# julilili42/hockey-env

Measured on NVIDIA B200. Metric: env-steps/sec, higher is better.
Workload: dtype f32

## Files before the change

hockey_env_b200/csrc/hk_lib.cu:

```cuda
#include <cuda_runtime.h>
#include <cstdio>
#include <cstdlib>
#include <cstring>
#include <algorithm>
#include <string>

#include "../../include/hockey_b200.h"
#include "hk_tick.cuh"
#if !defined(HK_TU_INLINE)
#include "hk_actor.cuh"
#endif

using namespace hk;

namespace {

__constant__ Scene c_scene;

thread_local std::string g_err;
int fail(int code, const std::string& msg) {
  g_err = msg;
  return code;
}
#define HK_CUDA(call)                                                                           \
// ... 30 lines not shown
  for (int k = 0; k < CORE_GROUPS; ++k) {
    float4 v = __ldcs(&core[(int64_t)k * n + i]);
    g[k] = F4{v.x, v.y, v.z, v.w};
  }
  groupsToEnv(g, e);
}
__device__ __forceinline__ void storeEnv(float4* __restrict__ core, int64_t n, int64_t i, const Env& e) {
  F4 g[CORE_GROUPS];
  envToGroups(e, g);
#pragma unroll
  for (int k = 0; k < CORE_GROUPS; ++k) __stcs(&core[(int64_t)k * n + i], make_float4(g[k].x, g[k].y, g[k].z, g[k].w));
}

__device__ __forceinline__ void flushInt(double* gstats, int slot, int v, int lane) {
  if (!__any_sync(0xffffffffu, v != 0)) return;
  int s = __reduce_add_sync(0xffffffffu, v);
  if (lane == 0 && s != 0) atomicAdd(&gstats[slot], (double)s);
}
__device__ __forceinline__ double warpSumD(double v) {
  for (int o = 16; o > 0; o >>= 1) v += __shfl_down_sync(0xffffffffu, v, o);
  return v;
}
constexpr int kStatsRows = 64;
__device__ __forceinline__ double* statsRow(double* gstats) { return gstats + HK_STATS_DIM * (blockIdx.x & (kStatsRows - 1)); }
__device__ __forceinline__ void flushStats(double* gstats, const TickStats& st) {
  const int lane = threadIdx.x & 31;
  flushInt(gstats, 4, st.steps, lane);
  flushInt(gstats, 11, st.velIters, lane);
  flushInt(gstats, 9, st.touch1, lane);
  flushInt(gstats, 10, st.touch2, lane);
  flushInt(gstats, 12, st.toi, lane);
  flushInt(gstats, 13, st.overflow, lane);
  if (__any_sync(0xffffffffu, st.episodes != 0)) {
    flushInt(gstats, 0, st.episodes, lane);
    flushInt(gstats, 1, st.wins, lane);
    flushInt(gstats, 2, st.losses, lane);
    flushInt(gstats, 3, st.draws, lane);
    flushInt(gstats, 8, st.len, lane);
    double a = warpSumD(st.ret1), b = warpSumD(st.ret2), c = warpSumD(st.ret1sq);
    if (lane == 0) {
      atomicAdd(&gstats[5], a);
      atomicAdd(&gstats[6], b);
      atomicAdd(&gstats[7], c);
    }
  }
}

}
namespace hkk {
struct KParams {
  float4* core;
  uint32_t* cache;
  double* stats;
  int32_t* queue;
  uint32_t* qctl;
  unsigned long long* phaseClk;
  float* actBuf;
  uint32_t* trace;
  int64_t n;
  int64_t env_id_offset;
  Config cfg;
};
}
using hkk::KParams;
#define HK_INL_DECLS                                                                                                              \
  cudaError_t setScene(const hk::Scene& S);                                                                                       \
  cudaError_t setMaxDynamicSmem(int bytes);                                                                                       \
  size_t staticSmemGeneral();                                                                                                     \
  void setCarveouts(int pctGeneral, int pctTouch);                                                                                \
  void launchGeneral1(unsigned grid, int block, size_t smem, cudaStream_t stream, const KParams& P, const hk::StepIO& io,         \
                      int unlimited, int lanesLog2, int firstClass, int phaseSync, int envWarps, int classWarps);                 \
  void launchTouch(unsigned grid, int block, cudaStream_t stream, const KParams& P, const hk::StepIO& io);
namespace hkinl { HK_INL_DECLS }
namespace hkinl256 { HK_INL_DECLS }
#if !defined(HK_INL_NS)
#define HK_INL_NS hkinl
#endif
namespace {

constexpr int kSlowBlock = 384;
constexpr int kTouchBlock = 384;

#if !defined(HK_TU_INLINE)
__global__ void __launch_bounds__(kBlock) k_create(KParams P) {
  __shared__ Scene S;
  stageScene(&S);
  int64_t i = (int64_t)blockIdx.x * blockDim.x + threadIdx.x;
  if (i >= P.n) return;
  Env e;
  envCreate(S, P.cfg, e, (uint64_t)(P.env_id_offset + i));
  storeEnv(P.core, P.n, i, e);
}

__global__ void __launch_bounds__(kBlock) k_reset(KParams P, const uint8_t* mask, const int8_t* one_starting, const int64_t* seeds,
                                                  const uint8_t* modes, float* obs) {
  __shared__ Scene S;
  stageScene(&S);
  int64_t i = (int64_t)blockIdx.x * blockDim.x + threadIdx.x;
  if (i >= P.n) return;
  if (mask && !mask[i]) return;
  Env e;
  loadEnv(P.core, P.n, i, e);
  envReset(S, P.cfg, e, (uint64_t)(P.env_id_offset + i), one_starting ? (int)one_starting[i] : -1, seeds ? seeds[i] : -1,
           modes ? (int)modes[i] : -1);
  storeEnv(P.core, P.n, i, e);
  if (obs) {
    float o[18];
    getObs(e, o);
    writeRow18(obs + 18 * i, o);
  }
}

__global__ void __launch_bounds__(kBlock) k_step(KParams P, StepIO io) {
  __shared__ Scene S;
  stageScene(&S);
  int64_t i = (int64_t)blockIdx.x * blockDim.x + threadIdx.x;
  TickStats st;
  tickStatsZero(st);
  if (i < P.n) {
    Env e;
    loadEnv(P.core, P.n, i, e);
    Cache cache;
    cache.base = P.cache + i;
    cache.stride = (size_t)P.n;
    envTick(S, P.cfg, cache, e, (uint64_t)(P.env_id_offset + i), (size_t)i, io, true, st);
    storeEnv(P.core, P.n, i, e);
  }
  flushStats(statsRow(P.stats), st);
}

#endif
enum { Q_CLASSES = 4, QC_DONE1 = 4, QC_COUNT2 = 5, QC_DONE2 = 6 };

#if !defined(HK_TU_INLINE)
constexpr int kFastWide = 512;
template <int MINB, int BLOCK>
__global__ void __launch_bounds__(BLOCK, MINB) k_fast(KParams P, StepIO io) {
  constexpr bool kStaged = BLOCK > kBlock;
  __shared__ Scene S;
  __shared__ __align__(16) float sRows[BLOCK / 32][32 * 18];
  stageScene(&S);
  const int64_t i = (int64_t)blockIdx.x * blockDim.x + threadIdx.x;
  const bool valid = i < P.n;
  TickStats st;
  tickStatsZero(st);
  bool ok = false, wroteFinal = false;
  int cls = 0;
  const bool stageRows = io.write != 0 && io.stageRows != 0;
  float* const myRows = sRows[threadIdx.x >> 5];
  if (!kStaged) {
    if (valid) {
      Env e;
      loadEnv(P.core, P.n, i, e);
      e.bailKind = 15;
      ok = envTickFast(S, P.cfg, e, (uint64_t)(P.env_id_offset + i), (size_t)i, io, io.write != 0, st, stageRows ? &wroteFinal : nullptr);
      if (ok) {
        storeEnv(P.core, P.n, i, e);
        if (stageRows) getObs(e, myRows + 18 * (threadIdx.x & 31));
      } else {
        tickStatsZero(st);
        cls = bailClass(e.bailKind);
      }
    }
  } else {
    Env e;
    float a[8];
    int had1 = 0, had2 = 0;
    const uint64_t env_id = (uint64_t)(P.env_id_offset + i);
    if (valid) {
      loadEnv(P.core, P.n, i, e);
      e.bailKind = 15;
      policyActions(P.cfg, e, env_id, io.action ? io.action + (size_t)io.stride * i : nullptr, io.pol1, pol2Of(io, (size_t)i), a);
      had1 = e.has1;
      had2 = e.has2;
    }
    __syncthreads();
    if (valid) {
      ok = envStepFast(S, P.cfg, e, a);
      if (!ok && io.actBuf) {
        float4* ab = reinterpret_cast<float4*>(io.actBuf + 8 * i);
        ab[0] = make_float4(a[0], a[1], a[2], a[3]);
        ab[1] = make_float4(a[4], a[5], a[6], a[7]);
      }
    }
    __syncthreads();
    if (valid) {
      if (ok) {
        tickFinish(S, P.cfg, e, env_id, (size_t)i, io, io.write != 0, st, had1, had2, stageRows ? &wroteFinal : nullptr);
        storeEnv(P.core, P.n, i, e);
        if (stageRows) getObs(e, myRows + 18 * (threadIdx.x & 31));
      } else {
        cls = bailClass(e.bailKind);
      }
    }
  }
  if (stageRows) {
    __syncwarp();
    const int64_t i0 = i - (threadIdx.x & 31);
    const unsigned okMask = __ballot_sync(0xffffffffu, ok), finMask = __ballot_sync(0xffffffffu, ok && !wroteFinal);
    if (okMask) warpStoreRows18(io.obs + 18 * i0, myRows, okMask);
    if (io.final_obs && finMask) warpStoreRows18(io.final_obs + 18 * i0, myRows, finMask);
  }
  const bool need = valid && !ok;
  const int lane = threadIdx.x & 31;
  if (__any_sync(0xffffffffu, need)) {
#pragma unroll
    for (int c = 0; c < Q_CLASSES; ++c) {
      const unsigned m = __ballot_sync(0xffffffffu, need && cls == c);
      if (m) {
        unsigned base = 0;
        if (lane == 0) base = atomicAdd(&P.qctl[c], (unsigned)__popc(m));
        base = __shfl_sync(0xffffffffu, base, 0);
        if (need && cls == c) P.queue[(int64_t)c * P.n + base + __popc(m & ((1u << lane) - 1u))] = (int32_t)i;
      }
    }
  }
  flushStats(statsRow(P.stats), st);
}

#endif
#if defined(HK_TU_INLINE)
__global__ void __launch_bounds__(kTouchBlock, 1) k_touch(KParams P, StepIO io) {
  __shared__ Scene S;
  stageScene(&S);
  const int lane = threadIdx.x & 31;
  const int64_t j = (int64_t)blockIdx.x * blockDim.x + threadIdx.x;
  const unsigned cnt = *((volatile uint32_t*)&P.qctl[0]);
  if ((int64_t)blockIdx.x * blockDim.x >= (int64_t)cnt) return;
  const bool valid = j < (int64_t)cnt;
  TickStats st;
  tickStatsZero(st);
  Env e;
  Cache cache;
  float a[8];
  int had1 = 0, had2 = 0;
  int64_t i = 0;
  bool live = false;
  const float h = (float)(1.0 / HK_FPS);
  if (valid) {
    i = P.queue[j];
    loadEnv(P.core, P.n, i, e);
    cache.base = P.cache + i;
    cache.stride = (size_t)P.n;
    const float4* ab = reinterpret_cast<const float4*>(io.actBuf + 8 * i);
    float4 lo = ab[0], hi = ab[1];
    a[0] = lo.x; a[1] = lo.y; a[2] = lo.z; a[3] = lo.w; a[4] = hi.x; a[5] = hi.y; a[6] = hi.z; a[7] = hi.w;
    e.bailKind = 15;
    policyAdvancePhases(P.cfg, e, (uint64_t)(P.env_id_offset + i), io.pol1, pol2Of(io, (size_t)i));
    had1 = e.has1;
    had2 = e.has2;
    envStepActions(S, P.cfg, e, a);
    e.sweepBudget = 1 << 20;
    e.allowToiEvents = true;
    e.aborted = false;
    live = worldStepTouchCollide(S, P.cfg, cache, e);
  }
  __syncthreads();
  if (live) live = worldStepTouchSolve(S, P.cfg, cache, e, h);
  __syncthreads();
  if (live) live = worldStepTouchFinish(S, cache, e);
  if (live) {
    envStepAfterWorld(e);
    tickFinish(S, P.cfg, e, (uint64_t)(P.env_id_offset + i), (size_t)i, io, io.write != 0, st, had1, had2);
    storeEnv(P.core, P.n, i, e);
  }
  const bool need = valid && !live;
  const unsigned m = __ballot_sync(0xffffffffu, need);
  if (m) {
    unsigned base = 0;
    if (lane == 0) base = atomicAdd(&P.qctl[Q_CLASSES - 1], (unsigned)__popc(m));
    base = __shfl_sync(0xffffffffu, base, 0);
    if (need) P.queue[(int64_t)(Q_CLASSES - 1) * P.n + base + __popc(m & ((1u << lane) - 1u))] = (int32_t)i;
  }
  flushStats(statsRow(P.stats), st);
}
#endif
constexpr int kMidSweeps = 24;
struct SolveTask {
  VC vcs[3];
  VelTriple v;
  int result, sweeps, kind;
};
struct Solve2Task {
  VC vc;
  Vel A, B;
  int result, sweeps;
};
struct Solve1Task {
  VC1 vc;
  Vel A, B;
  int result, sweeps;
};
constexpr int kMultiSlots = 24;
constexpr int kTasksPerLane = 3;
constexpr size_t kRawMulti = sizeof(SolveTask) * kMultiSlots;
__host__ __device__ constexpr int twoPointSlots(int envLanes) { return envLanes / 8 < 16 ? 16 : envLanes / 8; }
__host__ __device__ constexpr size_t rawBytes(int envLanes) {
  const size_t solve = kRawMulti + sizeof(Solve2Task) * (size_t)twoPointSlots(envLanes) + sizeof(Solve1Task) * (size_t)envLanes;
  const size_t toi = (sizeof(ToiTask) + sizeof(float)) * (size_t)envLanes * kTasksPerLane;
  return solve > toi ? solve : toi;
}
struct GenStamps {
  long long tc0, tc1, tc2, tc3, stampB, stampV, stampT, tf0, tfCommit, tfFinish, tfStore, tfFlush;
};
__device__ __forceinline__ long long clockAfterBarrier(const Scene& S) {
  const unsigned v = *reinterpret_cast<const volatile unsigned*>(&S.puckRadius);
  long long t = 0;
  if (v != 0xFFFFFFFFu) t = clock64();
  return t;
}
template <bool TEAM>
__device__ __forceinline__ void teamSync(int nthr) {
  if (TEAM) asm volatile("bar.sync 2, %0;" ::"r"(nthr) : "memory");
  else __syncthreads();
}
template <int TIER, bool TEAM>
__device__ __forceinline__ void generalTick(const KParams& P, const StepIO& io, const Scene& S, unsigned char* sRaw, const bool valid,
                                            const int64_t i, const int cls, const bool envWarp, const int64_t gw, const int unlimited,
                                            const int phaseSync, const int envWarps, const int nthr, const bool laneWrite,
                                            TickStats& st, bool& need, GenStamps& gs, unsigned long long* sSlowUnitP, unsigned* sFin) {
  const int envLanes = envWarps << 5;
  tickStatsZero(st);
  need = false;
  const int lane = threadIdx.x & 31;
  const int wib = threadIdx.x >> 5;
  Env e;
  Cache cache;
  cache.base = P.cache + i;
  cache.stride = (size_t)P.n;
  int had1 = 0, had2 = 0;
  const uint64_t env_id = (uint64_t)(P.env_id_offset + i);
  const float dt = (float)(1.0 / HK_FPS);
  long long& tc0 = gs.tc0; tc0 = clock64();
  if (valid) {
    loadEnv(P.core, P.n, i, e);
    float a[8];
    if (io.actBuf) {
      const float4* ab = reinterpret_cast<const float4*>(io.actBuf + 8 * i);
      float4 lo = ab[0], hi = ab[1];
      a[0] = lo.x; a[1] = lo.y; a[2] = lo.z; a[3] = lo.w; a[4] = hi.x; a[5] = hi.y; a[6] = hi.z; a[7] = hi.w;
      policyAdvancePhases(P.cfg, e, env_id, io.pol1, pol2Of(io, (size_t)i));
    } else {
      policyActions(P.cfg, e, env_id, io.action ? io.action + (size_t)io.stride * i : nullptr, io.pol1, pol2Of(io, (size_t)i), a);
    }
    had1 = e.has1;
    had2 = e.has2;
    e.sweepBudget = (TIER == 1 && !unlimited) ? kMidSweeps : (1 << 20);
    e.allowToiEvents = TIER != 1 || unlimited;
    e.aborted = false;
    envStepActions(S, P.cfg, e, a);
    worldStepCollide(S, P.cfg, cache, e);
  }
  const long long tw1 = clock64();
  if (phaseSync & 1) teamSync<TEAM>(nthr);
  long long& tc1 = gs.tc1; tc1 = clockAfterBarrier(S);
  IslandCtx ctx;
  ctx.nvc = 0;
  long long &stampB = gs.stampB, &stampV = gs.stampV, &stampT = gs.stampT;
  stampB = stampV = stampT = 0;
  if (valid) solveIslandsBegin(S, cache, e, dt, ctx);
  {
    SolveTask* mtasks = reinterpret_cast<SolveTask*>(sRaw);
    Solve2Task* s2tasks = reinterpret_cast<Solve2Task*>(sRaw + kRawMulti);
    const int cap2 = twoPointSlots(envLanes);
    Solve1Task* s1tasks = reinterpret_cast<Solve1Task*>(sRaw + kRawMulti + sizeof(Solve2Task) * (size_t)cap2);
    __shared__ int sKindCount[HK_MULTI_KINDS + 3];
    __shared__ unsigned short sList[2][kSlowBlock];
    __shared__ int sRound[5];
    if (threadIdx.x < HK_MULTI_KINDS + 3) sKindCount[threadIdx.x] = 0;
    if (threadIdx.x < 5) sRound[threadIdx.x] = 0;
    if (threadIdx.x == 0) *sSlowUnitP = 0;
    teamSync<TEAM>(nthr);
    stampB = clockAfterBarrier(S);
    const int nwarps = nthr >> 5;
    const int budget = (TIER == 1 && !unlimited) ? kMidSweeps : (1 << 20);
    const bool pool1 = (phaseSync & 8) != 0;
    int kind = 0, slot = 0;
    if (valid && ctx.nvc >= 2) {
      kind = solveKind(ctx.vcs, ctx.nvc);
      if (kind) {
        slot = atomicAdd(&sKindCount[HK_MULTI_KINDS + 2], 1);
        if (slot >= kMultiSlots) kind = 0;
        else atomicAdd(&sKindCount[kind - 1], 1);
      }
    } else if (valid && ctx.nvc == 1 && pool1) {
      kind = HK_MULTI_KINDS + ctx.vcs[0].count;
      slot = atomicAdd(&sKindCount[kind - 1], 1);
      if (kind == HK_MULTI_KINDS + 2 && slot >= cap2) kind = 0;
    }
    if (kind == HK_MULTI_KINDS + 1) {
      Solve1Task& t = s1tasks[slot];
      t.vc = vc1Of(ctx.vcs[0]);
      t.A = loadVel(e, ctx.vcs[0].bA);
      t.B = loadVel(e, ctx.vcs[0].bB);
    } else if (kind == HK_MULTI_KINDS + 2) {
      Solve2Task& t = s2tasks[slot];
      t.vc = ctx.vcs[0];
      t.A = loadVel(e, ctx.vcs[0].bA);
      t.B = loadVel(e, ctx.vcs[0].bB);
    } else if (kind) {
      SolveTask& t = mtasks[slot];
      t.kind = kind;
      for (int k = 0; k < ctx.nvc; ++k) t.vcs[k] = ctx.vcs[k];
      t.v.b0 = loadVel(e, 0);
      t.v.b1 = loadVel(e, 1);
      t.v.b2 = loadVel(e, 2);
    }
    teamSync<TEAM>(nthr);
    {
      const int n1 = sKindCount[HK_MULTI_KINDS], n2 = min(sKindCount[HK_MULTI_KINDS + 1], cap2);
      const int nMulti = min(sKindCount[HK_MULTI_KINDS + 2], kMultiSlots);
      int nm = 0, mk_[HK_MULTI_KINDS];
#pragma unroll
      for (int q = 0; q < HK_MULTI_KINDS; ++q) {
        const int k = q == 0 ? 4 : (q == 1 ? 6 : (q == 2 ? 7 : (q == 3 ? 8 : (q == 4 ? 2 : (q == 5 ? 3 : (q == 6 ? 5 : 1))))));
        if (sKindCount[k - 1] > 0) mk_[nm++] = k;
      }
      const int c2 = (n2 + 31) >> 5;
      int c1 = (n1 + 31) >> 5;
      const int spare = nwarps - nm - c2;
      if (spare > c1) c1 = min(spare, (n1 + 3) >> 2);
      const int units = (phaseSync & 16) ? nm + c2 : nm + c2 + c1;
      const int wHeavy = !(phaseSync & 16) || units == 0 || nwarps == 1 ? 0 : min(units, max(1, nwarps / 2));
      const int uStride = (phaseSync & 16) ? max(wHeavy, 1) : nwarps;
      const bool heavyWarp = !(phaseSync & 16) || wib < wHeavy || nwarps == 1;
      for (int r = 0, u = wib; heavyWarp && u < units; ++r, u = r * uStride + ((r & 1) ? uStride - 1 - wib : wib)) {
        const long long tu0 = P.trace ? clock64() : 0;
        int utype = 10;
        if (u < nm) {
          utype = mk_[u];
          const int k = mk_[u];
          const unsigned mine = __ballot_sync(0xffffffffu, lane < nMulti && mtasks[lane < nMulti ? lane : 0].kind == k);
          if (lane < __popc(mine)) {
            SolveTask& t = mtasks[__fns(mine, 0, lane + 1)];
            VelTriple v = t.v;
            int sweeps = 0;
            t.result = runVelocityIterationsKind(k, t.vcs, v, budget, 6 * 30, &sweeps);
            t.v = v;
            t.sweeps = sweeps;
          }
        } else if (u < nm + c2) {
          const int j = ((u - nm) << 5) + lane;
          if (j < n2) {
            Solve2Task& t = s2tasks[j];
            Vel A = t.A, B = t.B;
            int sweeps = 0;
            t.result = runVelocityIterations2Core(t.vc, A, B, budget, 6 * 30, &sweeps);
            t.A = A;
            t.B = B;
            t.sweeps = sweeps;
          }
        } else {
          const int c = u - nm - c2;
          const int lo = (int)(((long long)n1 * c) / c1), hi = (int)(((long long)n1 * (c + 1)) / c1);
          const int j = lo + lane;
          if (j < hi) {
            Solve1Task& t = s1tasks[j];
            Vel A = t.A, B = t.B;
            int sweeps = 0;
            t.result = runVelocityIterations1Core(t.vc, A, B, budget, 6 * 30, &sweeps);
            t.A = A;
            t.B = B;
            t.sweeps = sweeps;
          }
        }
        if (u >= nm && u < nm + c2) utype = 9;
        if (P.trace && lane == 0) atomicMax(sSlowUnitP, ((unsigned long long)(clock64() - tu0) << 8) | (unsigned)utype);
      }
      if ((phaseSync & 16) && wib >= wHeavy) {
        const long long tu0 = P.trace ? clock64() : 0;
        const int w1 = nwarps - wHeavy, myw = wib - wHeavy;
        int nA = n1, it0 = 0;
        for (int r = 0; r < 4 && nA > 0; ++r) {
          const int stop = r == 0 ? 12 : (r == 1 ? 24 : (r == 2 ? 48 : 6 * 30));
          const int chunks = (nA + 31) >> 5;
          for (int ch = myw; ch < chunks; ch += w1) {
            const int j = (ch << 5) + lane;
            if (j < nA) {
              const int idx = r == 0 ? j : (int)sList[r & 1][j];
              Solve1Task& t = s1tasks[idx];
              Vel A = t.A, B = t.B;
              int sweeps = 0;
              const int res = runVelocityIterations1Range(t.vc, A, B, budget, 6 * 30, it0, stop, &sweeps);
              t.A = A;
              t.B = B;
              if (res == HK_SOLVE_UNFINISHED) {
                sList[(r + 1) & 1][atomicAdd(&sRound[r + 1], 1)] = (unsigned short)idx;
              } else {
                t.result = res;
                t.sweeps = it0 + sweeps;
              }
            }
          }
          asm volatile("bar.sync 1, %0;" ::"r"(w1 * 32) : "memory");
          nA = sRound[r + 1];
          it0 = stop;
        }
        if (P.trace && lane == 0) atomicMax(sSlowUnitP, ((unsigned long long)(clock64() - tu0) << 8) | 10u);
      }
    }
    int itc = 0;
    {
      const long long tu0 = P.trace ? clock64() : 0;
      const bool inPlace = valid && ctx.nvc > 0 && !kind;
      if (inPlace) itc = runVelocityIterations(e, ctx.vcs, ctx.nvc, 6 * 30);
      if (P.trace && __any_sync(0xffffffffu, inPlace) && lane == 0) atomicMax(sSlowUnitP, ((unsigned long long)(clock64() - tu0) << 8) | 11u);
    }
    teamSync<TEAM>(nthr);
    stampV = clockAfterBarrier(S);
    if (kind == HK_MULTI_KINDS + 1) {
      const Solve1Task& t = s1tasks[slot];
      ctx.vcs[0].pt[0].ni = t.vc.ni;
      ctx.vcs[0].pt[0].ti = t.vc.ti;
      storeVel(e, ctx.vcs[0].bA, t.A);
      storeVel(e, ctx.vcs[0].bB, t.B);
      e.nVelIters += (uint32_t)t.sweeps;
      itc = t.result;
    } else if (kind == HK_MULTI_KINDS + 2) {
      const Solve2Task& t = s2tasks[slot];
      ctx.vcs[0].pt[0].ni = t.vc.pt[0].ni;
      ctx.vcs[0].pt[0].ti = t.vc.pt[0].ti;
      ctx.vcs[0].pt[1].ni = t.vc.pt[1].ni;
      ctx.vcs[0].pt[1].ti = t.vc.pt[1].ti;
      storeVel(e, ctx.vcs[0].bA, t.A);
      storeVel(e, ctx.vcs[0].bB, t.B);
      e.nVelIters += (uint32_t)t.sweeps;
      itc = t.result;
    } else if (kind) {
      const SolveTask& t = mtasks[slot];
      for (int k = 0; k < ctx.nvc; ++k) {
        ctx.vcs[k].pt[0].ni = t.vcs[k].pt[0].ni;
        ctx.vcs[k].pt[0].ti = t.vcs[k].pt[0].ti;
        if (ctx.vcs[k].count == 2) {
          ctx.vcs[k].pt[1].ni = t.vcs[k].pt[1].ni;
          ctx.vcs[k].pt[1].ti = t.vcs[k].pt[1].ti;
        }
      }
      storeVel(e, 0, t.v.b0);
      storeVel(e, 1, t.v.b1);
      storeVel(e, 2, t.v.b2);
      e.nVelIters += (uint32_t)t.sweeps;
      itc = t.result;
    }
    if (valid) solveIslandsEnd(S, e, dt, 2 * 30, ctx, itc);
  }
  const long long tw2 = clock64();
  if (phaseSync & 2) teamSync<TEAM>(nthr);
  long long& tc2 = gs.tc2; tc2 = clockAfterBarrier(S);
  const bool wantToi = valid && !e.aborted && (e.exist & HK_PAIRS_TOI);
  {
    ToiTask* sTasks = reinterpret_cast<ToiTask*>(sRaw);
    float* sAlpha = reinterpret_cast<float*>(sRaw + sizeof(ToiTask) * (size_t)envLanes * kTasksPerLane);
    __shared__ int sCount;
    if (threadIdx.x == 0) sCount = 0;
    teamSync<TEAM>(nthr);
    ToiTask mine[kTasksPerLane];
    int nMine = 0, base = 0;
    if (wantToi) {
      nMine = toiCollect(S, e, mine, kTasksPerLane);
      if (nMine > 0) {
        base = atomicAdd(&sCount, nMine);
        for (int k = 0; k < nMine; ++k) sTasks[base + k] = mine[k];
      }
    }
    teamSync<TEAM>(nthr);
    const int total = sCount;
    const int nwarps = nthr >> 5;
    for (int t = lane * nwarps + (threadIdx.x >> 5); t < total; t += nthr) sAlpha[t] = toiTaskRun(S, sTasks[t]);
    teamSync<TEAM>(nthr);
    stampT = clockAfterBarrier(S);
    for (int k = 0; k < nMine; ++k) {
      e.toiPre[mine[k].pid] = sAlpha[base + k];
      e.toiPreFlag |= 1u << mine[k].pid;
    }
  }
  const long long tw3a = clock64();
  if (wantToi) solveTOI(S, P.cfg, cache, e, dt, 6 * 30);
  const long long tw3 = clock64();
  if (P.trace && TIER == 1 && envWarp && lane == 0 && gw < P.n / 32 + 8) {
    uint32_t* w = P.trace + 4 * (size_t)gw;
    w[0] = (uint32_t)(tw1 - tc0);
    w[1] = (uint32_t)(tw2 - tc1);
    w[2] = (uint32_t)(tw3a - tc2);
    w[3] = (uint32_t)(tw3 - tw3a);
  }
  if (phaseSync & 4) teamSync<TEAM>(nthr);
  long long& tc3 = gs.tc3; tc3 = clockAfterBarrier(S);
  if (P.trace && (phaseSync & 4)) {
    __shared__ unsigned long long sMaxEval, sMaxEvent;
    if (threadIdx.x == 0) { sMaxEval = 0; sMaxEvent = 0; }
    teamSync<TEAM>(nthr);
    if (valid) {
      atomicMax(&sMaxEval, (unsigned long long)e.dbgEvalClk);
      atomicMax(&sMaxEvent, (unsigned long long)e.dbgEventClk);
    }
    teamSync<TEAM>(nthr);
    if (threadIdx.x == 0 && TIER == 1) {
      atomicAdd(&P.phaseClk[4], sMaxEval);
      atomicAdd(&P.phaseClk[5], sMaxEvent);
    }
  }
  if (P.trace && TIER == 1 && valid) {
    uint32_t* rec = P.trace + 4 * ((size_t)P.n / 32 + 8) + 2 * (size_t)i;
    rec[0] = (e.nVelIters & 0xFFFu) | ((e.nToiEvents & 0xFu) << 12) | ((uint32_t)(cls & 0xF) << 16) | ((e.dbgShape & 0xFFu) << 20) |
             (e.aborted ? 0x80000000u : 0u);
    rec[1] = (uint32_t)gw;
  }
  if (P.trace) {
    if (threadIdx.x < 4) sFin[threadIdx.x] = 0;
    teamSync<TEAM>(nthr);
  }
  if (io.waitFlag) {
    if (threadIdx.x == 0)
      while (*((volatile const uint32_t*)io.waitFlag) != io.waitValue) __nanosleep(200);
    teamSync<TEAM>(nthr);
  }
  const long long tf0 = clockAfterBarrier(S);
  long long tf1 = tf0, tf2 = tf0;
  gs.tf0 = tf0;
  if (valid) {
    if (!e.aborted) {
      worldStepFinish(cache, e);
      envStepAfterWorld(e);
      tf1 = clock64();
      if (P.trace && e.done) atomicAdd(&sFin[3], 1u);
      tickFinish(S, P.cfg, e, env_id, (size_t)i, io, laneWrite, st, had1, had2);
      tf2 = clock64();
      storeEnv(P.core, P.n, i, e);
    } else {
      need = true;
    }
  }
  __syncwarp();
  gs.tfCommit = tf1;
  gs.tfFinish = tf2;
  gs.tfStore = clock64();
  if (__any_sync(0xffffffffu, valid)) {
    if (TIER == 1 && !TEAM) {
      const unsigned m = __ballot_sync(0xffffffffu, need);
      if (m) {
        unsigned base = 0;
        if (lane == 0) base = atomicAdd(&P.qctl[QC_COUNT2], (unsigned)__popc(m));
        base = __shfl_sync(0xffffffffu, base, 0);
        if (need) P.queue[(int64_t)Q_CLASSES * P.n + base + __popc(m & ((1u << lane) - 1u))] = (int32_t)i;
      }
    }
    flushInt(statsRow(P.stats), 14, st.steps, lane);
    flushStats(statsRow(P.stats), st);
  }
  gs.tfFlush = clock64();
  if (P.trace && valid) {
    atomicMax(&sFin[0], (unsigned)(tf1 - tf0));
    atomicMax(&sFin[1], (unsigned)(tf2 - tf1));
    atomicMax(&sFin[2], (unsigned)(clock64() - tf2));
  }
}

template <int TIER>
#if !defined(HK_GENERAL_BOUND)
#define HK_GENERAL_BOUND kSlowBlock
#endif
__global__ void __launch_bounds__(HK_GENERAL_BOUND, 1) k_general(KParams P, StepIO io, int unlimited, int lanesLog2, int firstClass, int phaseSync, int envWarps, int classWarps) {
  __shared__ Scene S;
  extern __shared__ __align__(16) unsigned char sRaw[];
  stageScene(&S);
  const int lane = threadIdx.x & 31;
  const int wib = threadIdx.x >> 5;
  bool envWarp = wib < envWarps;
  int64_t gw = (int64_t)blockIdx.x * envWarps + wib;
  const int envLanes = envWarps << 5;
  int cls = 0;
  bool valid = false;
  int64_t i = 0;
  if (TIER == 1 && classWarps) {
    unsigned cnt[Q_CLASSES];
    int64_t nw[Q_CLASSES];
#pragma unroll
    for (int c = 0; c < Q_CLASSES; ++c) {
      cnt[c] = c < firstClass ? 0u : *((volatile uint32_t*)&P.qctl[c]);
      const int ll = (lanesLog2 >> (3 * c)) & 7;
      nw[c] = ((int64_t)cnt[c] + (1 << ll) - 1) >> ll;
    }
    int packed = classWarps;
    if (classWarps < 0) {
      const int maxW = envWarps, target = -classWarps;
      int b = 1;
      for (; b < maxW; ++b) {
        const int w0_ = min(2 * b, maxW);
        int64_t blocks = (nw[0] + w0_ - 1) / w0_;
#pragma unroll
        for (int c = 1; c < Q_CLASSES; ++c) blocks += (nw[c] + b - 1) / b;
        if (blocks <= target) break;
      }
      packed = min(2 * b, maxW) | (b << 4) | (b << 8) | (b << 12);
    }
    int64_t w0 = 0, b0 = 0;
    envWarp = false;
#pragma unroll
    for (int c = 0; c < Q_CLASSES; ++c) {
      const int ll = (lanesLog2 >> (3 * c)) & 7, lanes = 1 << ll;
      const int wpb = (packed >> (4 * c)) & 15;
      const int64_t nb = (nw[c] + wpb - 1) / wpb;
      if (!valid && (int64_t)blockIdx.x >= b0 && (int64_t)blockIdx.x < b0 + nb && wib < wpb) {
        const int64_t w = ((int64_t)blockIdx.x - b0) * wpb + wib;
        if (w < nw[c]) {
          envWarp = true;
          gw = w0 + w;
          const int64_t j = (w << ll) + lane;
          if (lane < lanes && j < (int64_t)cnt[c]) {
            valid = true;
            cls = c;
            i = P.queue[(int64_t)c * P.n + j];
          }
        }
      }
      w0 += nw[c];
      b0 += nb;
    }
  } else if (TIER == 1) {
    int64_t w0 = 0;
#pragma unroll
    for (int c = 0; c < Q_CLASSES; ++c) {
      const unsigned cnt = c < firstClass ? 0u : *((volatile uint32_t*)&P.qctl[c]);
      const int ll = (lanesLog2 >> (3 * c)) & 7, lanes = 1 << ll;
      const int64_t nw = ((int64_t)cnt + lanes - 1) >> ll;
      if (envWarp && !valid && gw >= w0 && gw < w0 + nw && lane < lanes) {
        const int64_t j = ((gw - w0) << ll) + lane;
        if (j < (int64_t)cnt) {
          valid = true;
          cls = c;
          i = P.queue[(int64_t)c * P.n + j];
        }
      }
      w0 += nw;
    }
  } else {
    const unsigned cnt = *((volatile uint32_t*)&P.qctl[QC_COUNT2]);
    const int ll = lanesLog2 & 7, lanes = 1 << ll;
    const int64_t j = (gw << ll) + lane;
    if (envWarp && lane < lanes && j < (int64_t)cnt) {
      valid = true;
      i = P.queue[(int64_t)Q_CLASSES * P.n + j];
    }
  }
  TickStats st;
  bool need = false;
  GenStamps gs;
  __shared__ unsigned long long sSlowUnit;
  __shared__ unsigned sFin[4];
  generalTick<TIER, false>(P, io, S, sRaw, valid, i, cls, envWarp, gw, unlimited, phaseSync, envWarps, (int)blockDim.x, io.write != 0, st,
                           need, gs, &sSlowUnit, sFin);
  const long long tc0 = gs.tc0, tc1 = gs.tc1, tc2 = gs.tc2, tc3 = gs.tc3, stampB = gs.stampB, stampV = gs.stampV, stampT = gs.stampT;

  __syncthreads();
  if (threadIdx.x == 0) {
    if (__any_sync(1u, valid) || true) {
      long long tc4 = clockAfterBarrier(S);
      if (P.trace && TIER == 1 && blockIdx.x < P.n / 32 + 8) {
        uint32_t* w = P.trace + 4 * ((size_t)P.n / 32 + 8) + 2 * (size_t)P.n + 16 * (size_t)blockIdx.x;
        w[0] = (uint32_t)(tc1 - tc0);
        w[1] = (uint32_t)(stampB - tc1);
        w[2] = (uint32_t)(stampV - stampB);
        w[3] = (uint32_t)(tc2 - stampV);
        w[4] = (uint32_t)(stampT - tc2);
        w[5] = (uint32_t)(tc3 - stampT);
        w[6] = (uint32_t)(tc4 - tc3);
        unsigned sm;
        asm volatile("mov.u32 %0, %%smid;" : "=r"(sm));
        w[7] = sm;
        unsigned long long gt;
        asm volatile("mov.u64 %0, %%globaltimer;" : "=l"(gt));
        w[8] = (uint32_t)gt;
        w[9] = (uint32_t)(tc4 - tc0);
        w[10] = (uint32_t)(sSlowUnit >> 8);
        w[11] = (uint32_t)(sSlowUnit & 0xFF);
        w[12] = sFin[0];
        w[13] = sFin[1];
        w[14] = sFin[2];
        w[15] = sFin[3];
      }
      if (!P.trace && TIER == 1) {
        atomicAdd(&P.phaseClk[8], (unsigned long long)(gs.tf0 - tc3));
        atomicAdd(&P.phaseClk[9], (unsigned long long)(gs.tfCommit - gs.tf0));
        atomicAdd(&P.phaseClk[10], (unsigned long long)(gs.tfFinish - gs.tfCommit));
        atomicAdd(&P.phaseClk[11], (unsigned long long)(gs.tfStore - gs.tfFinish));
        atomicAdd(&P.phaseClk[12], (unsigned long long)(gs.tfFlush - gs.tfStore));
        atomicAdd(&P.phaseClk[13], (unsigned long long)(tc4 - gs.tfFlush));
      }
      unsigned long long* pc = P.phaseClk + 4 * (TIER - 1);
      atomicAdd(&pc[0], (unsigned long long)(tc1 - tc0));
      atomicAdd(&pc[1], (unsigned long long)(tc2 - tc1));
      atomicAdd(&pc[2], (unsigned long long)(tc3 - tc2));
      atomicAdd(&pc[3], (unsigned long long)(tc4 - tc3));
    }
    __threadfence();
    unsigned t = atomicAdd(&P.qctl[TIER == 1 ? QC_DONE1 : QC_DONE2], 1u);
    if (t == gridDim.x - 1) {
      if (TIER == 1) {
        for (int c = 0; c < Q_CLASSES; ++c) P.qctl[c] = 0;
        P.qctl[QC_DONE1] = 0;
      } else {
        P.qctl[QC_COUNT2] = 0;
        P.qctl[QC_DONE2] = 0;
      }
      __threadfence();
    }
  }
}

#if defined(HK_TU_INLINE)
}
namespace HK_INL_NS {
cudaError_t setScene(const hk::Scene& S) { return cudaMemcpyToSymbol(c_scene, &S, sizeof(Scene)); }
cudaError_t setMaxDynamicSmem(int bytes) { return cudaFuncSetAttribute(k_general<1>, cudaFuncAttributeMaxDynamicSharedMemorySize, bytes); }
size_t staticSmemGeneral() {
  cudaFuncAttributes fa;
  return cudaFuncGetAttributes(&fa, k_general<1>) == cudaSuccess ? fa.sharedSizeBytes : sizeof(Scene) + 2048;
}
void setCarveouts(int pctGeneral, int pctTouch) {
  cudaFuncSetAttribute(k_general<1>, cudaFuncAttributePreferredSharedMemoryCarveout, pctGeneral);
  cudaFuncSetAttribute(k_touch, cudaFuncAttributePreferredSharedMemoryCarveout, pctTouch);
}
void launchGeneral1(unsigned grid, int block, size_t smem, cudaStream_t stream, const KParams& P, const hk::StepIO& io, int unlimited,
                    int lanesLog2, int firstClass, int phaseSync, int envWarps, int classWarps) {
  k_general<1><<<grid, block, smem, stream>>>(P, io, unlimited, lanesLog2, firstClass, phaseSync, envWarps, classWarps);
}
void launchTouch(unsigned grid, int block, cudaStream_t stream, const KParams& P, const hk::StepIO& io) {
  k_touch<<<grid, block, 0, stream>>>(P, io);
}
}
#else
__global__ void __launch_bounds__(kBlock) k_rollout(KParams P, StepIO io, int k_steps) {
  __shared__ Scene S;
  stageScene(&S);
  int64_t i = (int64_t)blockIdx.x * blockDim.x + threadIdx.x;
  TickStats st;
  tickStatsZero(st);
  if (i < P.n) {
    Env e;
    loadEnv(P.core, P.n, i, e);
    Cache cache;
    cache.base = P.cache + i;
    cache.stride = (size_t)P.n;
    for (int s = 0; s < k_steps; ++s)
      envTick(S, P.cfg, cache, e, (uint64_t)(P.env_id_offset + i), (size_t)i, io, s == k_steps - 1, st);
    storeEnv(P.core, P.n, i, e);
  }
  flushStats(statsRow(P.stats), st);
}

constexpr int kFusedChunk = 512;
struct FusedShared {
  int fastRing[kFusedChunk];
  int genRing[Q_CLASSES][kFusedChunk];
  int remaining[kFusedChunk];
  unsigned fastHead, fastTail, genHead[Q_CLASSES], genTail[Q_CLASSES];
  int doneCount, roundActive, batch;
  int asgClass[kSlowBlock / 32], asgStart[kSlowBlock / 32], asgCount[kSlowBlock / 32];
};
__device__ __forceinline__ void ringPush(int* ring, unsigned* tail, int j) {
  const unsigned slot = atomicAdd(tail, 1u) % kFusedChunk;
  while (atomicCAS(&ring[slot], -1, j) != -1) {}
}
__device__ __forceinline__ int ringTake(int* ring, unsigned pos) {
  const unsigned slot = pos % kFusedChunk;
  int j;
  while ((j = atomicExch(&ring[slot], -1)) < 0) {}
  return j;
}
__global__ void __launch_bounds__(kSlowBlock, 1) k_rollout_fused(KParams P, StepIO io, int k_steps, int phaseSync, int chunk, int nChunks, int fastRun) {
  __shared__ Scene S;
  extern __shared__ __align__(16) unsigned char sRaw[];
  __shared__ FusedShared F;
  __shared__ unsigned long long sSlowUnit;
  __shared__ unsigned sFin[4];
  stageScene(&S);
  const int lane = threadIdx.x & 31, wib = threadIdx.x >> 5;
  const int nwarps = blockDim.x >> 5;
  TickStats stFast;
  tickStatsZero(stFast);
  for (int c = blockIdx.x; c < nChunks; c += gridDim.x) {
    const int64_t lo = (int64_t)c * chunk;
    const int m = (int)(P.n - lo < (int64_t)chunk ? P.n - lo : (int64_t)chunk);
    for (int j = threadIdx.x; j < kFusedChunk; j += blockDim.x) {
      F.fastRing[j] = j < m ? j : -1;
      F.remaining[j] = k_steps;
#pragma unroll
      for (int q = 0; q < Q_CLASSES; ++q) F.genRing[q][j] = -1;
    }
    if (threadIdx.x == 0) {
      F.fastHead = 0;
      F.fastTail = (unsigned)m;
      for (int q = 0; q < Q_CLASSES; ++q) F.genHead[q] = F.genTail[q] = 0;
      F.doneCount = 0;
    }
    __syncthreads();
    for (;;) {
      if (threadIdx.x == 0) {
        const int due = (int)(F.fastTail - F.fastHead), waves = (due + blockDim.x - 1) / (int)blockDim.x;
        const int b = waves > 0 ? (due + nwarps * waves - 1) / (nwarps * waves) : 32;
        F.batch = b < 8 ? 8 : (b > 32 ? 32 : b);
      }
      __syncthreads();
      const long long tf0 = clock64();
      int batches = 0;
      for (;;) {
        int take = 0;
        unsigned h = 0;
        if (lane == 0) {
          for (;;) {
            const unsigned hh = *((volatile unsigned*)&F.fastHead), tt = *((volatile unsigned*)&F.fastTail);
            const int avail = (int)(tt - hh);
            if (avail <= 0) { take = -1; break; }
            const int want = avail < F.batch ? avail : F.batch;
            if (atomicCAS(&F.fastHead, hh, hh + (unsigned)want) == hh) { h = hh; take = want; break; }
          }
        }
        take = __shfl_sync(0xffffffffu, take, 0);
        h = __shfl_sync(0xffffffffu, h, 0);
        if (take < 0) break;
        ++batches;
        if (lane < take) {
          const int j = ringTake(F.fastRing, h + (unsigned)lane);
          const int64_t i = lo + j;
          const uint64_t env_id = (uint64_t)(P.env_id_offset + i);
          Env e;
          loadEnv(P.core, P.n, i, e);
          int rem = F.remaining[j];
          for (int it = 0;; ++it) {
            e.bailKind = 15;
            if (!envTickFast(S, P.cfg, e, env_id, (size_t)i, io, rem == 1 && io.obs != nullptr, stFast)) {
              F.remaining[j] = rem;
              const int q = bailClass(e.bailKind);
              ringPush(F.genRing[q], &F.genTail[q], j);
              break;
            }
            --rem;
            F4 g[CORE_GROUPS];
            envToGroups(e, g);
#pragma unroll
            for (int k = 0; k < CORE_GROUPS; ++k) P.core[(int64_t)k * P.n + i] = make_float4(g[k].x, g[k].y, g[k].z, g[k].w);
            if (rem == 0 || it + 1 >= fastRun) {
              F.remaining[j] = rem;
              __threadfence_block();
              if (rem > 0) ringPush(F.fastRing, &F.fastTail, j);
              else atomicAdd(&F.doneCount, 1);
              break;
            }
            groupsToEnv(g, e);
          }
        }
        __syncwarp();
      }
      __syncthreads();
      if (P.phaseClk && lane == 0) {
        atomicAdd(&P.phaseClk[4], (unsigned long long)batches);
        if (threadIdx.x == 0) {
          atomicAdd(&P.phaseClk[5], 1ull);
          atomicAdd(&P.phaseClk[6], (unsigned long long)(clock64() - tf0));
        }
      }
      if (F.doneCount >= m) break;
      for (;;) {
        const long long tr0 = clock64();
        if (threadIdx.x == 0) {
          int w = 0;
#pragma unroll
          for (int q = 0; q < Q_CLASSES; ++q) {
            int avail = (int)(F.genTail[q] - F.genHead[q]);
            while (avail > 0 && w < nwarps) {
              const int cnt = avail < 32 ? avail : 32;
              F.asgClass[w] = q;
              F.asgStart[w] = (int)F.genHead[q];
              F.asgCount[w] = cnt;
              F.genHead[q] += (unsigned)cnt;
              avail -= cnt;
              ++w;
            }
          }
          F.roundActive = w;
          for (; w < nwarps; ++w) F.asgCount[w] = 0;
        }
        __syncthreads();
        if (!F.roundActive) break;
        const int envWarps = F.roundActive;
        const int cnt = F.asgCount[wib], cls = F.asgClass[wib];
        const bool valid = lane < cnt;
        int j = 0;
        if (valid) j = ringTake(F.genRing[cls], (unsigned)F.asgStart[wib] + (unsigned)lane);
        const int64_t i = lo + j;
        bool need = false;
        GenStamps gs;
        TickStats st;
        generalTick<1, false>(P, io, S, sRaw, valid, i, cls, cnt > 0, (int64_t)wib, 1, phaseSync, envWarps, (int)blockDim.x,
                              valid && F.remaining[j] == 1 && io.obs != nullptr, st, need, gs, &sSlowUnit, sFin);
        if (valid) {
          const int rem = --F.remaining[j];
          if (rem > 0) ringPush(F.fastRing, &F.fastTail, j);
          else atomicAdd(&F.doneCount, 1);
        }
        __syncthreads();
        if (P.phaseClk) {
          if (lane == 0 && cnt > 0) atomicAdd(&P.phaseClk[1], (unsigned long long)cnt);
          if (threadIdx.x == 0) {
            atomicAdd(&P.phaseClk[0], 1ull);
            atomicAdd(&P.phaseClk[2], (unsigned long long)(clock64() - tr0));
          }
        }
      }
      if (F.doneCount >= m) break;
    }
    __syncthreads();
  }
  flushStats(statsRow(P.stats), stFast);
}

__global__ void __launch_bounds__(kBlock) k_get_obs(KParams P, float* obs, float* obs2) {
  int64_t i = (int64_t)blockIdx.x * blockDim.x + threadIdx.x;
  if (i >= P.n) return;
  Env e;
  loadEnv(P.core, P.n, i, e);
  float o[18];
  if (obs) {
    getObs(e, o);
    writeRow18(obs + 18 * i, o);
  }
  if (obs2) {
    getObs2(e, o);
    writeRow18(obs2 + 18 * i, o);
  }
}

__global__ void __launch_bounds__(kBlock) k_get_info(KParams P, float* info, float* info2) {
  int64_t i = (int64_t)blockIdx.x * blockDim.x + threadIdx.x;
  if (i >= P.n) return;
  Env e;
  loadEnv(P.core, P.n, i, e);
  double v[4];
  if (info) {
    getInfo(e, false, v);
    for (int k = 0; k < 4; ++k) info[4 * i + k] = (float)v[k];
  }
  if (info2) {
    getInfo(e, true, v);
    for (int k = 0; k < 4; ++k) info2[4 * i + k] = (float)v[k];
  }
}

__global__ void __launch_bounds__(kBlock) k_get_state(KParams P, uint32_t* rec) {
  int64_t i = (int64_t)blockIdx.x * blockDim.x + threadIdx.x;
  if (i >= P.n) return;
  Env e;
  loadEnv(P.core, P.n, i, e);
  Cache cache;
  cache.base = P.cache + i;
  cache.stride = (size_t)P.n;
  uint32_t* r = rec + (size_t)HK_STATE_WORDS * i;
  packRecord(e, cache, r);
  r[HK_S_MODE] = modeWord(e, P.cfg.mode);
}

__global__ void __launch_bounds__(kBlock) k_set_state(KParams P, const uint32_t* rec) {
  int64_t i = (int64_t)blockIdx.x * blockDim.x + threadIdx.x;
  if (i >= P.n) return;
  Env e;
  Cache cache;
  cache.base = P.cache + i;
  cache.stride = (size_t)P.n;
  const uint32_t* r = rec + (size_t)HK_STATE_WORDS * i;
  unpackRecord(r, e, cache);
  e.mode = modeOfWord(r[HK_S_MODE], P.cfg.mode);
  storeEnv(P.core, P.n, i, e);
}

__global__ void __launch_bounds__(kBlock) k_get_modes(KParams P, uint8_t* modes) {
  int64_t i = (int64_t)blockIdx.x * blockDim.x + threadIdx.x;
  if (i >= P.n) return;
  Env e;
  loadEnv(P.core, P.n, i, e);
  modes[i] = (uint8_t)e.mode;
}

__global__ void __launch_bounds__(kBlock) k_set_obs_state(KParams P, const float* obs18) {
  __shared__ Scene S;
  stageScene(&S);
  int64_t i = (int64_t)blockIdx.x * blockDim.x + threadIdx.x;
  if (i >= P.n) return;
  Env e;
  loadEnv(P.core, P.n, i, e);
  setObsState(S, e, obs18 + 18 * i, P.cfg.keep_mode);
  storeEnv(P.core, P.n, i, e);
}

}

static long long g_shapedFor = -1;

struct hk_env {
  int64_t n;
  int device;
  int64_t env_id_offset;
  Config cfg;
  float4* core;
  uint32_t* cache;
  double* stats;
  int32_t* queue;
  uint32_t* qctl;
  unsigned long long* phaseClk;
  float* actBuf;
  uint32_t* trace;
  const uint8_t* pol2v = nullptr;
  const uint8_t* resetModes = nullptr;
  bool fused = false;
  int fusedFastRun = 4;
  int sms = 148;
  int tiers;
  bool mono;
  KParams params() const {
    KParams P;
    P.core = core;
    P.cache = cache;
    P.stats = stats;
    P.queue = queue;
    P.qctl = qctl;
    P.phaseClk = phaseClk;
    P.actBuf = actBuf;
    P.trace = trace;
    P.n = n;
    P.env_id_offset = env_id_offset;
    P.cfg = cfg;
    return P;
  }
  unsigned grid() const { return (unsigned)((n + kBlock - 1) / kBlock); }
  unsigned gridSlow(int lanesPacked, int envWarps, int classWarpsPacked = 0) const {
    int lanesLog2 = 5;
    for (int c = 0; c < Q_CLASSES; ++c) lanesLog2 = std::min(lanesLog2, (lanesPacked >> (3 * c)) & 7);
    int64_t warps = ((n + (1 << lanesLog2) - 1) >> lanesLog2) + 4;
    if (classWarpsPacked < 0)
      return (unsigned)std::max<int64_t>(-classWarpsPacked, (warps + envWarps - 1) / envWarps + Q_CLASSES);
    if (classWarpsPacked > 0) {
      envWarps = 15;
      for (int c = 0; c < Q_CLASSES; ++c) envWarps = std::min(envWarps, (classWarpsPacked >> (4 * c)) & 15);
    }
    return (unsigned)((warps + envWarps - 1) / envWarps) + (classWarpsPacked ? Q_CLASSES : 0);
  }
  int envWarps1, block1;
  int classWarps1 = 0;
  int targetBlocks = 140;
  void shapeTier1() {
    const int maxWarps = kSlowBlock / 32;
    envWarps1 = tiers == 3 ? 6 : (n < 100000 ? 5 : maxWarps);
    block1 = envWarps1 * 32;
    if (const char* e = getenv("HK_ENV_WARPS")) envWarps1 = atoi(e);
    if (const char* e = getenv("HK_SLOW_BLOCK")) block1 = atoi(e) / 32 * 32;
    if (envWarps1 < 1) envWarps1 = 1;
    if (envWarps1 > maxWarps) envWarps1 = maxWarps;
    if (block1 < envWarps1 * 32) block1 = envWarps1 * 32;
    if (block1 > kSlowBlock) block1 = kSlowBlock;
    if (const char* e = getenv("HK_TARGET_BLOCKS")) targetBlocks = atoi(e);
    if (tiers == 2 && !getenv("HK_ENV_WARPS") && targetBlocks > 0) {
      envWarps1 = n <= 40000 ? 4 : (n <= 100000 ? 8 : maxWarps);
      if (const char* e = getenv("HK_AUTO_WARPS")) envWarps1 = std::min(maxWarps, std::max(1, atoi(e)));
      block1 = envWarps1 * 32;
      if (const char* e = getenv("HK_SLOW_BLOCK")) block1 = std::min(kSlowBlock, std::max(block1, atoi(e) / 32 * 32));
      classWarps1 = -targetBlocks;
    }
    if (const char* cw = getenv("HK_CLASS_WARPS")) {
      int packed = 0, c = 0, mx = 0;
      for (; c < Q_CLASSES; ++c) {
        const int v = cw[c] >= '1' && cw[c] <= '9' ? cw[c] - '0' : (cw[c] >= 'a' && cw[c] <= 'c' ? cw[c] - 'a' + 10 : 0);
        if (!v) break;
        packed |= v << (4 * c);
        mx = std::max(mx, v);
      }
      if (c == Q_CLASSES) {
        classWarps1 = packed;
        envWarps1 = mx;
        block1 = std::max(mx * 32, getenv("HK_SLOW_BLOCK") ? std::min(kSlowBlock, atoi(getenv("HK_SLOW_BLOCK")) / 32 * 32) : 0);
      } else if (cw[0] == '0') {
        classWarps1 = 0;
        envWarps1 = n < 100000 ? 5 : maxWarps;
        block1 = envWarps1 * 32;
      }
    }
  }
  int blockTier2() const {
    int64_t b = ((int64_t)(0.06 * (double)n) / (2 * 148) + 31) / 32 * 32;
    if (b < 64) b = 64;
    if (b > kSlowBlock) b = kSlowBlock;
    return (int)b;
  }
  int lanes1, lanes2;
  bool touch;
  int phaseSync;
  int launches;
  bool carveout = true;
  long long shapeKey() const { return carveout ? ((long long)device << 56) ^ ((long long)block1 << 40) ^ ((long long)classWarps1 << 44) ^ (long long)gridSlow(lanes1, envWarps1, classWarps1) : -2; }
  int fastBlock = kBlock;
  bool fastWide = false;
  int fastWideBlock = kFastWide;
  size_t staticSmem = sizeof(Scene) + 2048;
  size_t fastSmem = sizeof(Scene) + sizeof(float) * kBlock * 18;
  void shapeSharedMemory() const {
    if (!carveout) return;
    auto pct = [](size_t bytes) { return (int)std::min<size_t>(100, (bytes * 100 + 228 * 1024 - 1) / (228 * 1024)); };
    const size_t stat = staticSmem;
    const int perSm1 = std::max(1, std::min(65536 / (168 * block1), (int)((gridSlow(lanes1, envWarps1, classWarps1) + 147) / 148)));
    const int perSmAuto = std::max(1, (targetBlocks + sms - 1) / sms);
    hkinl::setCarveouts(pct((rawBytes(envWarps1 * 32) + stat) * (classWarps1 < 0 ? perSmAuto : perSm1)), pct(stat));
    hkinl256::setCarveouts(pct((rawBytes(envWarps1 * 32) + stat) * (classWarps1 < 0 ? perSmAuto : perSm1)), pct(stat));
    cudaFuncSetAttribute(k_fast<4, kBlock>, cudaFuncAttributePreferredSharedMemoryCarveout, pct((fastSmem + 1024) * 4));
    cudaFuncSetAttribute(k_fast<5, kBlock>, cudaFuncAttributePreferredSharedMemoryCarveout, pct((fastSmem + 1024) * 5));
    cudaFuncSetAttribute(k_fast<1, kFastWide>, cudaFuncAttributePreferredSharedMemoryCarveout, pct(sizeof(Scene) + sizeof(float) * kFastWide * 18 + 1024));
    cudaFuncSetAttribute(k_rollout_fused, cudaFuncAttributePreferredSharedMemoryCarveout, pct(rawBytes(kSlowBlock) + stat + sizeof(FusedShared)));
  }
  enum { kTimedSteps = 2048, kEventsPerStep = 5 };
  cudaEvent_t* events = nullptr;
  mutable int timedSteps = 0;
  void stamp(int k, cudaStream_t stream) const {
    if (events && timedSteps < kTimedSteps) cudaEventRecord(events[timedSteps * kEventsPerStep + k], stream);
  }
  cudaStream_t sideStream = nullptr;
  cudaEvent_t evTiers = nullptr, evCopy = nullptr;
  uint32_t* flagDev = nullptr;
  uint32_t* seqHost = nullptr;
  uint32_t hostTick = 0;
  void launchCascade(const StepIO& io, cudaStream_t stream, const StepIO* ioGeneral = nullptr, void (*between)(const hk_env*, cudaStream_t, void*) = nullptr,
                     void* betweenArg = nullptr) const {
    if (g_shapedFor != shapeKey()) {
      shapeSharedMemory();
      g_shapedFor = shapeKey();
    }
    if (trace) cudaMemsetAsync(trace, 0, sizeof(uint32_t) * (20 * ((size_t)n / 32 + 8) + 2 * (size_t)n), stream);
    stamp(0, stream);
    if (fastWide) k_fast<1, kFastWide><<<(unsigned)((n + fastWideBlock - 1) / fastWideBlock), fastWideBlock, 0, stream>>>(params(), io);
    else if (n < 100000) k_fast<4, kBlock><<<(unsigned)((n + fastBlock - 1) / fastBlock), fastBlock, 0, stream>>>(params(), io);
    else k_fast<5, kBlock><<<(unsigned)((n + fastBlock - 1) / fastBlock), fastBlock, 0, stream>>>(params(), io);
    stamp(1, stream);
    if (touch) hkinl::launchTouch((unsigned)((n + kTouchBlock - 1) / kTouchBlock), kTouchBlock, stream, params(), io);
    stamp(2, stream);
    if (between) between(this, stream, betweenArg);
    const StepIO& iog = ioGeneral ? *ioGeneral : io;
    const int b2 = blockTier2(), w2 = b2 / 32;
    (block1 <= 256 ? hkinl256::launchGeneral1 : hkinl::launchGeneral1)(gridSlow(lanes1, envWarps1, classWarps1), block1, rawBytes(envWarps1 * 32),
                                                                       stream, params(), iog, tiers == 2 ? 1 : 0, lanes1, touch ? 1 : 0, phaseSync,
                                                                       envWarps1, classWarps1);
    stamp(3, stream);
    if (tiers == 3) k_general<2><<<gridSlow(lanes2, w2), b2, rawBytes(b2), stream>>>(params(), iog, 1, lanes2, 0, phaseSync, w2, 0);
    stamp(4, stream);
    if (events && timedSteps < kTimedSteps) ++timedSteps;
  }
};

static bool validPolicy(int p) { return p >= HK_POLICY_EXTERNAL && p <= HK_POLICY_ZERO; }

__global__ void k_sum_stats(const double* rows, double* out) {
  double s = 0.0;
  for (int r = 0; r < kStatsRows; ++r) s += rows[HK_STATS_DIM * r + threadIdx.x];
  out[threadIdx.x] = s;
}

__global__ void k_check_codes(const uint8_t* codes, int64_t n, int maxCode, int* bad) {
  int64_t i = (int64_t)blockIdx.x * blockDim.x + threadIdx.x;
  if (i < n && codes[i] > maxCode) atomicAdd(bad, 1);
}
static int checkCodes(const hk_env* h, const uint8_t* codes_dev, int maxCode, const char* msg) {
  DeviceGuard guard(h->device);
  int* bad = nullptr;
  int hostBad = 0;
  HK_CUDA(cudaMalloc(&bad, sizeof(int)));
  cudaMemset(bad, 0, sizeof(int));
  k_check_codes<<<h->grid(), kBlock>>>(codes_dev, h->n, maxCode, bad);
  cudaError_t err = cudaMemcpy(&hostBad, bad, sizeof(int), cudaMemcpyDeviceToHost);
  cudaFree(bad);
  HK_CUDA(err);
  return hostBad ? fail(HK_E_INVALID, msg) : HK_OK;
}

extern "C" {

const char* hk_last_error(void) { return g_err.c_str(); }
const char* hk_version(void) { return "hockey_b200 0.1 (sm_100a, fmad=false)"; }

int hk_create(hk_env** out, int64_t n_envs, int mode, int keep_mode, int device, uint64_t seed, int64_t env_id_offset) {
  if (!out) return fail(HK_E_INVALID, "hk_create: out is NULL");
  *out = nullptr;
  if (n_envs <= 0) return fail(HK_E_INVALID, "hk_create: n_envs must be positive");
  if (mode < HK_MODE_NORMAL || mode > HK_MODE_TRAIN_DEFENSE)
    return fail(HK_E_INVALID, std::to_string(mode) + " is not a valid value for Mode");
  int count = 0;
  if (cudaGetDeviceCount(&count) != cudaSuccess || count == 0)
    return fail(HK_E_NODEVICE, "hk_create: no CUDA device available (this library has no CPU fallback)");
  if (device < 0 || device >= count) return fail(HK_E_INVALID, "hk_create: bad device index");
  DeviceGuard guard(device);
  if (!guard.ok) return fail(HK_E_CUDA, "hk_create: cannot select device");
  hk_env* h = new hk_env();
  h->n = n_envs;
  h->device = device;
  h->env_id_offset = env_id_offset;
  h->cfg.mode = mode;
  h->cfg.keep_mode = keep_mode ? 1 : 0;
  h->cfg.max_timesteps = maxTimesteps(mode);
  h->cfg.seed = seed;
  h->core = nullptr;
  h->cache = nullptr;
  h->stats = nullptr;
  h->queue = nullptr;
  h->qctl = nullptr;
  h->phaseClk = nullptr;
  h->actBuf = nullptr;
  h->trace = nullptr;
  {
    const char* m = getenv("HK_MONO");
    h->mono = m && m[0] == '1';
    const char* t = getenv("HK_TIERS");
    h->tiers = 2;
    if (t && (t[0] == '2' || t[0] == '3')) h->tiers = t[0] - '0';
    h->lanes1 = 5;
    h->lanes2 = 5;
    if (const char* l1 = getenv("HK_LANES1")) h->lanes1 = atoi(l1);
    if (const char* l2 = getenv("HK_LANES2")) h->lanes2 = atoi(l2);
    if (h->lanes1 < 0 || h->lanes1 > 5) h->lanes1 = 5;
    if (h->lanes2 < 0 || h->lanes2 > 5) h->lanes2 = 5;
    h->lanes1 *= 01111;
    h->lanes2 *= 01111;
    if (n_envs >= 100000 && n_envs < 200000 && !getenv("HK_LANES1")) h->lanes1 = 5 | (5 << 3) | (4 << 6) | (4 << 9);
    if (const char* cl = getenv("HK_CLASS_LANES")) {
      int packed = 0, c = 0;
      for (; c < Q_CLASSES && cl[c] >= '0' && cl[c] <= '5'; ++c) packed |= (cl[c] - '0') << (3 * c);
      if (c == Q_CLASSES) h->lanes1 = packed;
    }
    const char* tt = getenv("HK_TOUCH");
    h->touch = n_envs >= 750000;
    if (tt && (tt[0] == '0' || tt[0] == '1')) h->touch = tt[0] == '1';
    if (const char* co = getenv("HK_CARVEOUT")) h->carveout = co[0] != '0';
    if (const char* fb = getenv("HK_FAST_BLOCK")) h->fastBlock = std::min(kBlock, std::max(32, atoi(fb) / 32 * 32));
    h->fastWide = n_envs >= 16000;
    if (const char* fw = getenv("HK_FAST_WIDE")) h->fastWide = fw[0] == '1';
    h->phaseSync = 31;
    if (const char* ps = getenv("HK_PHASE_SYNC")) h->phaseSync = atoi(ps) & 31;
    int sms = 148;
    if (cudaDeviceGetAttribute(&sms, cudaDevAttrMultiProcessorCount, device) != cudaSuccess || sms < 16) sms = 148;
    {
      const int64_t waves = (n_envs + (int64_t)sms * kFastWide - 1) / ((int64_t)sms * kFastWide);
      const int64_t per = (n_envs + sms * waves - 1) / (sms * waves);
      h->fastWideBlock = (int)std::min<int64_t>(kFastWide, std::max<int64_t>(128, (per + 31) / 32 * 32));
      if (const char* fb = getenv("HK_FAST_WIDE_BLOCK")) h->fastWideBlock = std::min(kFastWide, std::max(32, atoi(fb) / 32 * 32));
    }
    cudaFuncAttributes fa;
    h->staticSmem = hkinl::staticSmemGeneral();
    if (cudaFuncGetAttributes(&fa, k_fast<4, kBlock>) == cudaSuccess) h->fastSmem = fa.sharedSizeBytes;
    h->sms = sms;
    if (const char* f = getenv("HK_FUSED")) h->fused = f[0] != '0';
    if (const char* g = getenv("HK_FUSED_FAST_RUN")) h->fusedFastRun = std::max(1, atoi(g));
    h->targetBlocks = sms;
    h->shapeTier1();
    h->launches = h->mono ? 1 : 2 + (h->touch ? 1 : 0) + (h->tiers == 3 ? 1 : 0);
  }
  Scene S;
  std::memset(&S, 0, sizeof(S));
  scene_build::build(&S);
  cudaError_t err = cudaMemcpyToSymbol(c_scene, &S, sizeof(Scene));
  if (err == cudaSuccess) err = hkinl::setScene(S);
  if (err == cudaSuccess) err = hkinl::setMaxDynamicSmem((int)rawBytes(kSlowBlock));
  if (err == cudaSuccess) err = hkinl256::setScene(S);
  if (err == cudaSuccess) err = hkinl256::setMaxDynamicSmem((int)rawBytes(256));
  if (err == cudaSuccess) err = cudaFuncSetAttribute(k_general<2>, cudaFuncAttributeMaxDynamicSharedMemorySize, (int)rawBytes(kSlowBlock));
  if (err == cudaSuccess) err = cudaFuncSetAttribute(k_rollout_fused, cudaFuncAttributeMaxDynamicSharedMemorySize, (int)rawBytes(kSlowBlock));
  if (err == cudaSuccess) err = cudaMalloc(&h->core, sizeof(float4) * CORE_GROUPS * (size_t)n_envs);
  if (err == cudaSuccess) err = cudaMalloc(&h->cache, sizeof(uint32_t) * 6 * N_PAIRS * (size_t)n_envs);
  if (err == cudaSuccess) err = cudaMalloc(&h->stats, sizeof(double) * HK_STATS_DIM * (kStatsRows + 1));
  if (err == cudaSuccess) err = cudaMalloc(&h->queue, sizeof(int32_t) * 5 * (size_t)n_envs);
  if (err == cudaSuccess) err = cudaMalloc(&h->qctl, sizeof(uint32_t) * 8);
  if (err == cudaSuccess) err = cudaMemset(h->qctl, 0, sizeof(uint32_t) * 8);
  if (err == cudaSuccess) err = cudaMalloc(&h->actBuf, sizeof(float) * 8 * (size_t)n_envs);
  if (err == cudaSuccess) err = cudaMalloc(&h->phaseClk, sizeof(unsigned long long) * 16);
  if (err == cudaSuccess) err = cudaMemset(h->phaseClk, 0, sizeof(unsigned long long) * 16);
  if (err == cudaSuccess && getenv("HK_LANE_TRACE")) err = cudaMalloc(&h->trace, sizeof(uint32_t) * (20 * ((size_t)n_envs / 32 + 8) + 2 * (size_t)n_envs));
  if (err == cudaSuccess) err = cudaMemset(h->cache, 0, sizeof(uint32_t) * 6 * N_PAIRS * (size_t)n_envs);
  if (err == cudaSuccess) err = cudaMemset(h->stats, 0, sizeof(double) * HK_STATS_DIM * (kStatsRows + 1));
  if (err == cudaSuccess) {
    k_create<<<h->grid(), kBlock>>>(h->params());
    err = cudaGetLastError();
  }
  if (err == cudaSuccess) err = cudaDeviceSynchronize();
  if (err != cudaSuccess) {
    std::string msg = std::string("hk_create: ") + cudaGetErrorString(err);
    cudaFree(h->core);
    cudaFree(h->cache);
    cudaFree(h->stats);
    cudaFree(h->queue);
    cudaFree(h->qctl);
    cudaFree(h->phaseClk);
    cudaFree(h->actBuf);
    cudaFree(h->trace);
    delete h;
    return fail(HK_E_CUDA, msg);
  }
  *out = h;
  return HK_OK;
}

int hk_destroy(hk_env* h) {
  if (!h) return HK_OK;
  DeviceGuard guard(h->device);
  cudaFree(h->core);
  cudaFree(h->cache);
  cudaFree(h->stats);
  cudaFree(h->queue);
  cudaFree(h->qctl);
  cudaFree(h->phaseClk);
  cudaFree(h->actBuf);
  cudaFree(h->trace);
  if (h->events) {
    for (int k = 0; k < hk_env::kTimedSteps * hk_env::kEventsPerStep; ++k) cudaEventDestroy(h->events[k]);
    delete[] h->events;
  }
  if (h->sideStream) {
    cudaStreamDestroy(h->sideStream);
    cudaEventDestroy(h->evTiers);
    cudaEventDestroy(h->evCopy);
    cudaFree(h->flagDev);
    cudaFreeHost(h->seqHost);
  }
  delete h;
  return HK_OK;
}

int64_t hk_num_envs(const hk_env* h) { return h ? h->n : 0; }

int hk_reset_seeded(hk_env* h, const uint8_t* mask_dev, const int8_t* one_starting_dev, const int64_t* seeds_dev, float* obs_dev,
                    void* stream) {
  if (!h) return fail(HK_E_INVALID, "hk_reset: NULL handle");
  DeviceGuard guard(h->device);
  k_reset<<<h->grid(), kBlock, 0, (cudaStream_t)stream>>>(h->params(), mask_dev, one_starting_dev, seeds_dev, h->resetModes, obs_dev);
  HK_CUDA(cudaGetLastError());
  return HK_OK;
}

int hk_reset(hk_env* h, const uint8_t* mask_dev, const int8_t* one_starting_dev, float* obs_dev, void* stream) {
  return hk_reset_seeded(h, mask_dev, one_starting_dev, nullptr, obs_dev, stream);
}

int hk_step(hk_env* h, const float* action_dev, int action_stride, int p1_policy, int p2_policy, int flags, float* obs_dev,
            float* obs2_dev, float* reward_dev, float* reward2_dev, uint8_t* done_dev, float* info_dev, float* info2_dev,
            float* final_obs_dev, void* stream) {
  if (!h) return fail(HK_E_INVALID, "hk_step: NULL handle");
  const bool perEnv = p2_policy == HK_POLICY_PER_ENV;
  if (!validPolicy(p1_policy) || !(validPolicy(p2_policy) || perEnv)) return fail(HK_E_INVALID, "hk_step: invalid policy id");
  if (perEnv && !h->pol2v) return fail(HK_E_INVALID, "hk_step: HK_POLICY_PER_ENV without hk_set_opponent_policies");
  if (!obs_dev) return fail(HK_E_INVALID, "hk_step: obs_dev is required");
  if ((((uintptr_t)info_dev | (uintptr_t)info2_dev) & 15u) != 0) return fail(HK_E_INVALID, "hk_step: info tensors must be 16-byte aligned");
  if ((((uintptr_t)obs_dev | (uintptr_t)obs2_dev | (uintptr_t)final_obs_dev) & 7u) != 0)
    return fail(HK_E_INVALID, "hk_step: observation tensors must be 8-byte aligned");
  if ((p1_policy == HK_POLICY_EXTERNAL || p2_policy == HK_POLICY_EXTERNAL) && !action_dev)
    return fail(HK_E_INVALID, "hk_step: action_dev is NULL but a policy is EXTERNAL");
  if (p1_policy == HK_POLICY_EXTERNAL && action_stride < 4) return fail(HK_E_INVALID, "hk_step: action_stride < 4");
  if (p2_policy == HK_POLICY_EXTERNAL && action_stride < 8)
    return fail(HK_E_INVALID, "hk_step: player 2 EXTERNAL needs action_stride >= 8");
  if (perEnv && (!action_dev || action_stride < 8))
    return fail(HK_E_INVALID, "hk_step: HK_POLICY_PER_ENV needs action_dev with action_stride >= 8");
  DeviceGuard guard(h->device);
  StepIO io;
  io.action = action_dev;
  io.stride = action_stride;
  io.pol1 = p1_policy;
  io.pol2 = perEnv ? HK_POLICY_ZERO : p2_policy;
  io.pol2v = perEnv ? h->pol2v : nullptr;
  io.resetModes = h->resetModes;
  io.flags = flags;
  io.obs = obs_dev;
  io.obs2 = obs2_dev;
  io.reward = reward_dev;
  io.reward2 = reward2_dev;
  io.done = done_dev;
  io.info = info_dev;
  io.info2 = info2_dev;
  io.final_obs = final_obs_dev;
  io.write = 1;
  io.actBuf = nullptr;
  io.waitFlag = nullptr;
  io.waitValue = 0;
  io.stageRows = (((uintptr_t)obs_dev | (uintptr_t)final_obs_dev) & 15u) == 0 ? 1 : 0;
  if (h->mono) {
    k_step<<<h->grid(), kBlock, 0, (cudaStream_t)stream>>>(h->params(), io);
  } else {
    io.actBuf = h->actBuf;
    h->launchCascade(io, (cudaStream_t)stream);
  }
  HK_CUDA(cudaGetLastError());
  return HK_OK;
}

static int64_t recordLayout(int64_t n, int with_final_obs, int64_t off[5]) {
  auto up = [](int64_t x) { return (x + 255) / 256 * 256; };
  int64_t t = 0;
  off[0] = t; t += up(72 * n);
  off[1] = t; t += up(4 * n);
  off[2] = t; t += up(16 * n);
  off[3] = t; t += up(n);
  off[4] = t;
  if (with_final_obs) t += up(72 * n);
  return t;
}
int64_t hk_host_record_bytes(int64_t n_envs, int with_final_obs, int64_t* offsets5) {
  int64_t off[5];
  const int64_t t = recordLayout(n_envs, with_final_obs, off);
  if (offsets5) for (int k = 0; k < 5; ++k) offsets5[k] = off[k];
  return t;
}
static StepIO recordIO(const StepIO& base, uint8_t* rec, const int64_t off[5], int with_final_obs) {
  StepIO io = base;
  io.obs = reinterpret_cast<float*>(rec + off[0]);
  io.reward = reinterpret_cast<float*>(rec + off[1]);
  io.info = reinterpret_cast<float*>(rec + off[2]);
  io.done = rec + off[3];
  io.final_obs = with_final_obs ? reinterpret_cast<float*>(rec + off[4]) : nullptr;
  io.obs2 = io.reward2 = io.info2 = nullptr;
  return io;
}
struct HostCopyArgs {
  uint8_t* recDev;
  uint8_t* recHost;
  int64_t bytes;
};
static void copyFastRows(const hk_env* h, cudaStream_t stream, void* argp) {
  const HostCopyArgs* a = static_cast<const HostCopyArgs*>(argp);
  cudaEventRecord(h->evTiers, stream);
  cudaStreamWaitEvent(h->sideStream, h->evTiers, 0);
  cudaMemcpyAsync(a->recHost, a->recDev, (size_t)a->bytes, cudaMemcpyDeviceToHost, h->sideStream);
  cudaMemcpyAsync(h->flagDev, h->seqHost + (h->hostTick & 0xFFFFu), sizeof(uint32_t), cudaMemcpyHostToDevice, h->sideStream);
  cudaEventRecord(h->evCopy, h->sideStream);
}

int hk_step_host(hk_env* h, const float* action_host, int action_stride, int p1_policy, int p2_policy, int flags, float* action_dev,
                 uint8_t* record_dev, uint8_t* record_host, int with_final_obs, void* stream) {
  if (!h) return fail(HK_E_INVALID, "hk_step_host: NULL handle");
  if (!record_dev || !record_host) return fail(HK_E_INVALID, "hk_step_host: record_dev and record_host are required");
  const bool perEnv = p2_policy == HK_POLICY_PER_ENV;
  if (!validPolicy(p1_policy) || !(validPolicy(p2_policy) || perEnv)) return fail(HK_E_INVALID, "hk_step_host: invalid policy id");
  if (perEnv && !h->pol2v) return fail(HK_E_INVALID, "hk_step_host: HK_POLICY_PER_ENV without hk_set_opponent_policies");
  const bool ext = p1_policy == HK_POLICY_EXTERNAL || p2_policy == HK_POLICY_EXTERNAL || perEnv;
  if (ext && (!action_host || !action_dev)) return fail(HK_E_INVALID, "hk_step_host: action buffers are NULL but a policy is EXTERNAL");
  if (ext && (action_stride < 4 || ((p2_policy == HK_POLICY_EXTERNAL || perEnv) && action_stride < 8)))
    return fail(HK_E_INVALID, "hk_step_host: action_stride too small for the EXTERNAL policies");
  if ((((uintptr_t)record_dev | (uintptr_t)record_host) & 15u) != 0) return fail(HK_E_INVALID, "hk_step_host: records must be 16-byte aligned");
  DeviceGuard guard(h->device);
  cudaStream_t st = (cudaStream_t)stream;
  if (!h->sideStream) {
    HK_CUDA(cudaStreamCreateWithFlags(&h->sideStream, cudaStreamNonBlocking));
    HK_CUDA(cudaEventCreateWithFlags(&h->evTiers, cudaEventDisableTiming));
    HK_CUDA(cudaEventCreateWithFlags(&h->evCopy, cudaEventDisableTiming));
    HK_CUDA(cudaMalloc(&h->flagDev, sizeof(uint32_t)));
    HK_CUDA(cudaMemset(h->flagDev, 0xFF, sizeof(uint32_t)));
    HK_CUDA(cudaMallocHost(&h->seqHost, sizeof(uint32_t) * 65536));
    for (uint32_t k = 0; k < 65536; ++k) h->seqHost[k] = k;
  }
  int64_t off[5];
  const int64_t bytes = recordLayout(h->n, with_final_obs, off);
  if (ext) HK_CUDA(cudaMemcpyAsync(action_dev, action_host, sizeof(float) * (size_t)action_stride * (size_t)h->n, cudaMemcpyHostToDevice, st));
  StepIO io;
  std::memset(&io, 0, sizeof(io));
  io.action = ext ? action_dev : nullptr;
  io.stride = action_stride;
  io.pol1 = p1_policy;
  io.pol2 = perEnv ? HK_POLICY_ZERO : p2_policy;
  io.pol2v = perEnv ? h->pol2v : nullptr;
  io.resetModes = h->resetModes;
  io.flags = flags;
  io.write = 1;
  StepIO ioDev = recordIO(io, record_dev, off, with_final_obs);
  ioDev.stageRows = 1;
  if (h->mono) {
    k_step<<<h->grid(), kBlock, 0, st>>>(h->params(), ioDev);
    HK_CUDA(cudaMemcpyAsync(record_host, record_dev, (size_t)bytes, cudaMemcpyDeviceToHost, st));
  } else {
    ioDev.actBuf = h->actBuf;
    ++h->hostTick;
    StepIO ioHost = recordIO(ioDev, record_host, off, with_final_obs);
    ioHost.waitFlag = h->flagDev;
    ioHost.waitValue = h->hostTick & 0xFFFFu;
    HostCopyArgs args{record_dev, record_host, bytes};
    h->launchCascade(ioDev, st, &ioHost, copyFastRows, &args);
    HK_CUDA(cudaStreamWaitEvent(st, h->evCopy, 0));
  }
  HK_CUDA(cudaGetLastError());
  return HK_OK;
}

int hk_set_opponent_policies(hk_env* h, const uint8_t* codes_dev) {
  if (!h) return fail(HK_E_INVALID, "hk_set_opponent_policies: NULL handle");
  if (codes_dev) {
    const int rc = checkCodes(h, codes_dev, HK_POLICY_ZERO, "hk_set_opponent_policies: codes must be HK_POLICY_EXTERNAL..HK_POLICY_ZERO");
    if (rc != HK_OK) return rc;
  }
  h->pol2v = codes_dev;
  return HK_OK;
}

int hk_set_reset_modes(hk_env* h, const uint8_t* modes_dev) {
  if (!h) return fail(HK_E_INVALID, "hk_set_reset_modes: NULL handle");
  if (modes_dev) {
    const int rc = checkCodes(h, modes_dev, HK_MODE_TRAIN_DEFENSE, "hk_set_reset_modes: modes must be HK_MODE_NORMAL..HK_MODE_TRAIN_DEFENSE");
    if (rc != HK_OK) return rc;
  }
  h->resetModes = modes_dev;
  return HK_OK;
}

int hk_get_modes(hk_env* h, uint8_t* modes_dev, void* stream) {
  if (!h || !modes_dev) return fail(HK_E_INVALID, "hk_get_modes: NULL argument");
  DeviceGuard guard(h->device);
  k_get_modes<<<h->grid(), kBlock, 0, (cudaStream_t)stream>>>(h->params(), modes_dev);
  HK_CUDA(cudaGetLastError());
  return HK_OK;
}

int hk_rollout(hk_env* h, int k_steps, int p1_policy, int p2_policy, float* obs_dev, void* stream) {
  if (!h) return fail(HK_E_INVALID, "hk_rollout: NULL handle");
  if (k_steps <= 0) return fail(HK_E_INVALID, "hk_rollout: k_steps must be positive");
  if (!validPolicy(p1_policy) || !validPolicy(p2_policy) || p1_policy == HK_POLICY_EXTERNAL || p2_policy == HK_POLICY_EXTERNAL)
    return fail(HK_E_INVALID, "hk_rollout: policies must be in-kernel (not EXTERNAL)");
  DeviceGuard guard(h->device);
  StepIO io;
  std::memset(&io, 0, sizeof(io));
  io.pol1 = p1_policy;
  io.pol2 = p2_policy;
  io.resetModes = h->resetModes;
  io.flags = HK_STEP_AUTORESET;
  io.obs = obs_dev;
  if (h->mono) {
    io.write = 1;
    k_rollout<<<h->grid(), kBlock, 0, (cudaStream_t)stream>>>(h->params(), io, k_steps);
  } else if (h->fused) {
    io.actBuf = h->actBuf;
    io.write = obs_dev ? 1 : 0;
    KParams P = h->params();
    P.trace = nullptr;
    int64_t chunk = (h->n + h->sms - 1) / h->sms;
    if (chunk > kFusedChunk) chunk = kFusedChunk;
    const int64_t nChunks = (h->n + chunk - 1) / chunk;
    k_rollout_fused<<<(unsigned)std::min<int64_t>(nChunks, h->sms), kSlowBlock, rawBytes(kSlowBlock), (cudaStream_t)stream>>>(
        P, io, k_steps, h->phaseSync, (int)chunk, (int)nChunks, h->fusedFastRun);
  } else {
    io.actBuf = h->actBuf;
    for (int s = 0; s < k_steps; ++s) {
      io.write = (s == k_steps - 1 && obs_dev) ? 1 : 0;
      h->launchCascade(io, (cudaStream_t)stream);
    }
  }
  HK_CUDA(cudaGetLastError());
  return HK_OK;
}

int hk_get_obs(hk_env* h, float* obs_dev, float* obs2_dev, void* stream) {
  if (!h) return fail(HK_E_INVALID, "hk_get_obs: NULL handle");
  DeviceGuard guard(h->device);
  k_get_obs<<<h->grid(), kBlock, 0, (cudaStream_t)stream>>>(h->params(), obs_dev, obs2_dev);
  HK_CUDA(cudaGetLastError());
  return HK_OK;
}

int hk_get_info(hk_env* h, float* info_dev, float* info2_dev, void* stream) {
  if (!h) return fail(HK_E_INVALID, "hk_get_info: NULL handle");
  DeviceGuard guard(h->device);
  k_get_info<<<h->grid(), kBlock, 0, (cudaStream_t)stream>>>(h->params(), info_dev, info2_dev);
  HK_CUDA(cudaGetLastError());
  return HK_OK;
}

int hk_get_state(hk_env* h, uint32_t* state_dev, void* stream) {
  if (!h || !state_dev) return fail(HK_E_INVALID, "hk_get_state: NULL argument");
  DeviceGuard guard(h->device);
  k_get_state<<<h->grid(), kBlock, 0, (cudaStream_t)stream>>>(h->params(), state_dev);
  HK_CUDA(cudaGetLastError());
  return HK_OK;
}

int hk_set_state(hk_env* h, const uint32_t* state_dev, void* stream) {
  if (!h || !state_dev) return fail(HK_E_INVALID, "hk_set_state: NULL argument");
  DeviceGuard guard(h->device);
  k_set_state<<<h->grid(), kBlock, 0, (cudaStream_t)stream>>>(h->params(), state_dev);
  HK_CUDA(cudaGetLastError());
  return HK_OK;
}

int hk_set_obs_state(hk_env* h, const float* obs18_dev, void* stream) {
  if (!h || !obs18_dev) return fail(HK_E_INVALID, "hk_set_obs_state: NULL argument");
  DeviceGuard guard(h->device);
  k_set_obs_state<<<h->grid(), kBlock, 0, (cudaStream_t)stream>>>(h->params(), obs18_dev);
  HK_CUDA(cudaGetLastError());
  return HK_OK;
}

int hk_get_stats(hk_env* h, double* out_host, void* stream) {
  if (!h || !out_host) return fail(HK_E_INVALID, "hk_get_stats: NULL argument");
  DeviceGuard guard(h->device);
  double* sum = h->stats + HK_STATS_DIM * kStatsRows;
  k_sum_stats<<<1, HK_STATS_DIM, 0, (cudaStream_t)stream>>>(h->stats, sum);
  HK_CUDA(cudaMemcpyAsync(out_host, sum, sizeof(double) * HK_STATS_DIM, cudaMemcpyDeviceToHost, (cudaStream_t)stream));
  HK_CUDA(cudaStreamSynchronize((cudaStream_t)stream));
  return HK_OK;
}

int hk_clear_stats(hk_env* h, void* stream) {
  if (!h) return fail(HK_E_INVALID, "hk_clear_stats: NULL handle");
  DeviceGuard guard(h->device);
  HK_CUDA(cudaMemsetAsync(h->stats, 0, sizeof(double) * HK_STATS_DIM * (kStatsRows + 1), (cudaStream_t)stream));
  return HK_OK;
}

int hk_copy_stats(hk_env* h, double* dst_dev, void* stream) {
  if (!h || !dst_dev) return fail(HK_E_INVALID, "hk_copy_stats: NULL argument");
  DeviceGuard guard(h->device);
  k_sum_stats<<<1, HK_STATS_DIM, 0, (cudaStream_t)stream>>>(h->stats, dst_dev);
  HK_CUDA(cudaGetLastError());
  return HK_OK;
}

int hk_debug_phase_cycles(hk_env* h, double* out_host8) {
  if (!h || !out_host8) return fail(HK_E_INVALID, "hk_debug_phase_cycles: NULL argument");
  DeviceGuard guard(h->device);
  unsigned long long v[16];
  HK_CUDA(cudaMemcpy(v, h->phaseClk, sizeof(v), cudaMemcpyDeviceToHost));
  for (int k = 0; k < 8; ++k) out_host8[k] = (double)v[k];
  return HK_OK;
}

int hk_debug_finish_cycles(hk_env* h, double* out_host6) {
  if (!h || !out_host6) return fail(HK_E_INVALID, "hk_debug_finish_cycles: NULL argument");
  DeviceGuard guard(h->device);
  unsigned long long v[16];
  HK_CUDA(cudaMemcpy(v, h->phaseClk, sizeof(v), cudaMemcpyDeviceToHost));
  for (int k = 0; k < 6; ++k) out_host6[k] = (double)v[8 + k];
  return HK_OK;
}

int hk_debug_lane_trace(hk_env* h, uint32_t* out_host, int64_t n_words) {
  if (!h || !out_host) return fail(HK_E_INVALID, "hk_debug_lane_trace: NULL argument");
  if (!h->trace) return fail(HK_E_INVALID, "hk_debug_lane_trace: create the env with HK_LANE_TRACE=1");
  const int64_t have = 20 * (h->n / 32 + 8) + 2 * h->n;
  DeviceGuard guard(h->device);
  HK_CUDA(cudaMemcpy(out_host, h->trace, sizeof(uint32_t) * (size_t)(n_words < have ? n_words : have), cudaMemcpyDeviceToHost));
  return HK_OK;
}

int hk_actor_param_bytes(void) { return hk_actor::kParamBytes; }

int hk_actor_forward(const void* params_dev, const float* obs_dev, float* act_dev, int act_stride, int64_t n, int device, void* stream) {
  if (!params_dev || !obs_dev || !act_dev) return fail(HK_E_INVALID, "hk_actor_forward: NULL argument");
  if (n <= 0 || act_stride < hk_actor::kAct) return fail(HK_E_INVALID, "hk_actor_forward: n must be positive and act_stride >= 4");
  if ((((uintptr_t)params_dev) & 15u) || (((uintptr_t)obs_dev) & 7u)) return fail(HK_E_INVALID, "hk_actor_forward: params need 16-byte, obs 8-byte alignment");
  int count = 0;
  if (cudaGetDeviceCount(&count) != cudaSuccess || count == 0) return fail(HK_E_NODEVICE, "hk_actor_forward: no CUDA device (there is no CPU fallback)");
  if (device < 0 || device >= count) return fail(HK_E_INVALID, "hk_actor_forward: bad device index");
  DeviceGuard guard(device);
  static bool configured[64] = {false};
  if (!configured[device & 63]) {
    HK_CUDA(cudaFuncSetAttribute(hk_actor::k_actor_mlp, cudaFuncAttributeMaxDynamicSharedMemorySize, hk_actor::kSmemBytes));
    configured[device & 63] = true;
  }
  int sms = 148;
  if (cudaDeviceGetAttribute(&sms, cudaDevAttrMultiProcessorCount, device) != cudaSuccess || sms < 1) sms = 148;
  const int64_t tiles = (n + hk_actor::kRows - 1) / hk_actor::kRows;
  hk_actor::k_actor_mlp<<<(unsigned)std::min<int64_t>(tiles, sms), hk_actor::kThreads, hk_actor::kSmemBytes, (cudaStream_t)stream>>>(
      (const unsigned char*)params_dev, obs_dev, act_dev, act_stride, (long long)n);
  HK_CUDA(cudaGetLastError());
  return HK_OK;
}

int64_t hk_actor_pool_scratch_bytes(int64_t n, int k) {
  if (n <= 0 || n > INT32_MAX || k < 1 || k > hk_actor::kPoolMaxK)
    return fail(HK_E_INVALID, "hk_actor_pool_scratch_bytes: n must be in [1, 2^31 - 1] and k in [1, 4096]");
  return 4 * hk_actor::poolScratchWords(n, k);
}

int hk_actor_forward_pool(const void* params_dev, int k, const int32_t* choice_dev, const float* obs_dev, float* act_dev,
                          int act_stride, int64_t n, void* scratch_dev, int device, void* stream) {
  using namespace hk_actor;
  if (!params_dev || !choice_dev || !obs_dev || !act_dev || !scratch_dev) return fail(HK_E_INVALID, "hk_actor_forward_pool: NULL argument");
  if (n <= 0 || n > INT32_MAX || act_stride < kAct)
    return fail(HK_E_INVALID, "hk_actor_forward_pool: n must be in [1, 2^31 - 1] and act_stride >= 4");
  if (k < 1 || k > kPoolMaxK) return fail(HK_E_INVALID, "hk_actor_forward_pool: k must be in [1, 4096]");
  if ((((uintptr_t)params_dev) & 15u) || (((uintptr_t)obs_dev) & 7u) || (((uintptr_t)choice_dev) & 3u) || (((uintptr_t)scratch_dev) & 15u))
    return fail(HK_E_INVALID, "hk_actor_forward_pool: params and scratch need 16-byte, obs 8-byte, choice 4-byte alignment");
  int count = 0;
  if (cudaGetDeviceCount(&count) != cudaSuccess || count == 0) return fail(HK_E_NODEVICE, "hk_actor_forward_pool: no CUDA device (there is no CPU fallback)");
  if (device < 0 || device >= count) return fail(HK_E_INVALID, "hk_actor_forward_pool: bad device index");
  DeviceGuard guard(device);
  static bool configured[64] = {false};
  if (!configured[device & 63]) {
    HK_CUDA(cudaFuncSetAttribute(k_actor_pool_mlp, cudaFuncAttributeMaxDynamicSharedMemorySize, kSmemBytes));
    configured[device & 63] = true;
  }
  int sms = 148;
  if (cudaDeviceGetAttribute(&sms, cudaDevAttrMultiProcessorCount, device) != cudaSuccess || sms < 1) sms = 148;
  cudaStream_t st = (cudaStream_t)stream;
  int32_t* scratch = (int32_t*)scratch_dev;
  HK_CUDA(cudaMemsetAsync(scratch, 0, sizeof(int32_t) * (size_t)k, st));
  const int64_t chunks = (n + kPoolThreads * kPoolItems - 1) / (kPoolThreads * kPoolItems);
  const unsigned histBlocks = (unsigned)std::min<int64_t>(chunks, 4 * (int64_t)sms);
  k_pool_count<<<histBlocks, kPoolThreads, sizeof(int32_t) * (size_t)k, st>>>(choice_dev, (long long)n, k, scratch);
  k_pool_scan<<<1, kScanThreads, 0, st>>>(scratch, k);
  k_pool_scatter<<<histBlocks, kPoolThreads, 2 * sizeof(int32_t) * (size_t)k, st>>>(choice_dev, (long long)n, k, scratch);
  const int64_t grid = std::min<int64_t>(sms, (n + kRows - 1) / kRows + k);
  k_actor_pool_mlp<<<(unsigned)grid, kThreads, kSmemBytes, st>>>((const unsigned char*)params_dev, k, scratch, obs_dev, act_dev, act_stride);
  HK_CUDA(cudaGetLastError());
  return HK_OK;
}

int hk_launches_per_step(const hk_env* h) { return h ? h->launches : 0; }

int hk_kernel_timing(hk_env* h, int enable) {
  if (!h) return fail(HK_E_INVALID, "hk_kernel_timing: NULL handle");
  DeviceGuard guard(h->device);
  const int total = hk_env::kTimedSteps * hk_env::kEventsPerStep;
  if (enable && !h->events) {
    h->events = new cudaEvent_t[total];
    for (int k = 0; k < total; ++k) HK_CUDA(cudaEventCreate(&h->events[k]));
  } else if (!enable && h->events) {
    for (int k = 0; k < total; ++k) cudaEventDestroy(h->events[k]);
    delete[] h->events;
    h->events = nullptr;
  }
  h->timedSteps = 0;
  return HK_OK;
}

int hk_kernel_times(hk_env* h, double* out_ms4, int64_t* steps_out) {
  if (!h || !out_ms4) return fail(HK_E_INVALID, "hk_kernel_times: NULL argument");
  if (!h->events) return fail(HK_E_INVALID, "hk_kernel_times: call hk_kernel_timing(env, 1) first");
  DeviceGuard guard(h->device);
  HK_CUDA(cudaDeviceSynchronize());
  for (int k = 0; k < 4; ++k) out_ms4[k] = 0.0;
  for (int s = 0; s < h->timedSteps; ++s)
    for (int k = 0; k < 4; ++k) {
      float ms = 0.0f;
      HK_CUDA(cudaEventElapsedTime(&ms, h->events[s * hk_env::kEventsPerStep + k], h->events[s * hk_env::kEventsPerStep + k + 1]));
      out_ms4[k] += (double)ms;
    }
  if (steps_out) *steps_out = h->timedSteps;
  h->timedSteps = 0;
  return HK_OK;
}

int hk_stats_device_ptr(hk_env* h, double** out_dev) {
  if (!h || !out_dev) return fail(HK_E_INVALID, "hk_stats_device_ptr: NULL argument");
  DeviceGuard guard(h->device);
  double* sum = h->stats + HK_STATS_DIM * kStatsRows;
  k_sum_stats<<<1, HK_STATS_DIM>>>(h->stats, sum);
  HK_CUDA(cudaGetLastError());
  *out_dev = sum;
  return HK_OK;
}

}
#endif
```

hockey_env_b200/csrc/hk_world.cuh:

```cuda
#pragma once
#include "hk_collide.cuh"

namespace hk {

#if defined(HK_FAST_DEBUG) && !defined(__CUDA_ARCH__)
extern long long g_iter_hist[2][182];
extern long long g_nvc_hist[16];
extern long long g_period_hist[16];
extern long long g_toi_dbg[16];
#define HK_TOI_DBG(k) g_toi_dbg[k]++
#define HK_ITER_HIST(w, n) g_iter_hist[w][n]++
#define HK_NVC_HIST(n) g_nvc_hist[n]++
#else
#define HK_ITER_HIST(w, n)
#define HK_NVC_HIST(n)
#define HK_TOI_DBG(k)
#endif

enum { MAX_MANIFOLDS = 8, MAX_CLIST = 12 };

struct Body {
  V2 p;
  Rot q;
  V2 c0, c;
// ... 1553 lines not shown
          icIsl[nic] = (unsigned char)nIsl;
          ++nic;
        } else {
          e.nOverflow++;
        }
        inIsland |= bit;
        int bA = fixtureBody(S.pairFA[pid]), bB = fixtureBody(S.pairFB[pid]);
        int other = (bA == bi) ? bB : bA;
        if (other < 0) continue;
        if (e.b[other].island) continue;
        stack[sp++] = other;
        e.b[other].island = true;
      }
    }
    islBodies[nIsl++] = bm;
  }
  ctx.nIsl = nIsl;
  Rot* q0 = ctx.q0;
  for (int bi = 0; bi < 3; ++bi) {
    Body& b = e.b[bi];
    q0[bi] = b.q;
    if (!b.island) continue;
    b.c0 = b.c;
    b.a0 = b.a;
    b.v += h * (1.0f * mk(0.0f, 0.0f) + S.invMass[bi] * b.f);
    b.w += h * S.invI[bi] * b.tq;
    b.v *= fclamp(1.0f - h * b.ldamp, 0.0f, 1.0f);
    b.w *= fclamp(1.0f - h * b.adamp, 0.0f, 1.0f);
  }
  VC* vcs = ctx.vcs;
  int nvc = 0;
  for (int k = 0; k < nic; ++k) {
    int pid = ic[k];
    int slot = findSlot(e, pid);
    if (slot < 0) {
      if (e.nmf >= MAX_MANIFOLDS) {
        e.nOverflow++;
        continue;
      }
      slot = e.nmf++;
      e.mfPid[slot] = pid;
      evaluateManifold(S, e, pid, &e.mf[slot]);
      int oldCount = getCount(e, pid);
      for (int i = 0; i < e.mf[slot].count; ++i) {
        e.mf[slot].ni[i] = 0.0f;
        e.mf[slot].ti[i] = 0.0f;
        for (int j = 0; j < oldCount; ++j)
          if (cache.at(pid, j) == e.mf[slot].key[i]) {
            e.mf[slot].ni[i] = u2f(cache.at(pid, 2 + 2 * j));
            e.mf[slot].ti[i] = u2f(cache.at(pid, 3 + 2 * j));
            break;
          }
      }
    }
    if (e.mf[slot].count == 0) continue;
    ic[nvc] = pid;
    icIsl[nvc] = icIsl[k];
    initConstraint(S, e, pid, slot, true, &vcs[nvc]);
    ++nvc;
  }
  {
    int npts = 0;
    for (int k = 0; k < nvc; ++k) npts += vcs[k].count;
    e.dbgShape = (uint32_t)nvc | ((uint32_t)npts << 4);
  }
  ctx.nvc = nvc;
  for (int k = 0; k < nvc; ++k) warmStartConstraint(e, vcs[k]);
}
HK_HD_NOINLINE void solveIslandsEnd(const Scene& S, Env& e, float h, int posIters, IslandCtx& ctx, int itc) {
  const int nvc = ctx.nvc, nIsl = ctx.nIsl;
  VC* vcs = ctx.vcs;
  const int* ic = ctx.ic;
  const unsigned char* icIsl = ctx.icIsl;
  const uint32_t* islBodies = ctx.islBodies;
  const Rot* q0 = ctx.q0;
  if (nvc > 0) {
    if (itc < 0) {
      e.aborted = true;
      return;
    }
    HK_ITER_HIST(0, itc);
    HK_NVC_HIST(nvc);
    for (int k = 0; k < nvc; ++k) {
      Manifold& m = e.mf[vcs[k].slot];
      for (int j = 0; j < vcs[k].count; ++j) {
        m.ni[j] = vcs[k].pt[j].ni;
        m.ti[j] = vcs[k].pt[j].ti;
      }
    }
  }
  for (int bi = 0; bi < 3; ++bi)
    if (e.b[bi].island) integratePosition(e.b[bi], h);
  uint32_t islSolved = 0;
  {
    uint32_t withContacts = 0;
    for (int k = 0; k < nvc; ++k) withContacts |= 1u << icIsl[k];
    islSolved = ~withContacts;
    uint32_t active = withContacts;
    for (int it = 0; it < posIters && active; ++it) {
      float minSep[3] = {0.0f, 0.0f, 0.0f};
      for (int k = 0; k < nvc; ++k) {
        int isl = icIsl[k];
        if (!((active >> isl) & 1u)) continue;
        const Manifold& m = e.mf[vcs[k].slot];
        minSep[isl] = fmin2(minSep[isl], solvePositionConstraint(S, e, ic[k], m, m.count, false));
      }
      for (int isl = 0; isl < nIsl; ++isl) {
        if (!((active >> isl) & 1u)) continue;
        if (minSep[isl] >= -3.0f * HK_LINEAR_SLOP) {
          active &= ~(1u << isl);
          islSolved |= 1u << isl;
        }
      }
    }
  }
  for (int bi = 0; bi < 3; ++bi)
    if (e.b[bi].island) syncTransform(S, e.b[bi], bi);
  for (int isl = 0; isl < nIsl; ++isl) {
    const uint32_t bm = islBodies[isl];
    float minSleepTime = HK_MAXFLOAT;
    const float linTolSqr = HK_LINEAR_SLEEP_TOL * HK_LINEAR_SLEEP_TOL;
    const float angTolSqr = HK_ANGULAR_SLEEP_TOL * HK_ANGULAR_SLEEP_TOL;
    for (int bi = 0; bi < 3; ++bi) {
      if (!((bm >> bi) & 1u)) continue;
      Body& b = e.b[bi];
      if (b.w * b.w > angTolSqr || dot(b.v, b.v) > linTolSqr) {
        b.sleep = 0.0f;
        minSleepTime = 0.0f;
      } else {
        b.sleep += h;
        minSleepTime = fmin2(minSleepTime, b.sleep);
      }
    }
    if (minSleepTime >= HK_TIME_TO_SLEEP && ((islSolved >> isl) & 1u)) {
      for (int bi = 0; bi < 3; ++bi)
        if ((bm >> bi) & 1u) setAwake(e.b[bi], false);
    }
  }
  for (int bi = 2; bi >= 0; --bi)
    if (e.b[bi].island) synchronizeFixturesQ0(S, e, bi, q0[bi]);
  findNewContacts(S, e);
}
HK_HD_NOINLINE void solveIslands(const Scene& S, const Config& cfg, const Cache& cache, Env& e, float h, int velIters, int posIters) {
  (void)cfg;
  IslandCtx ctx;
  solveIslandsBegin(S, cache, e, h, ctx);
  const int itc = ctx.nvc > 0 ? runVelocityIterations(e, ctx.vcs, ctx.nvc, velIters) : 0;
  solveIslandsEnd(S, e, h, posIters, ctx, itc);
}

HK_HD Sweep bodySweep(const Scene& S, const Body& b, int bi) {
  Sweep s;
  s.lc = mk(S.lcx[bi], S.lcy[bi]);
  s.c0 = b.c0;
  s.c = b.c;
  s.a0 = b.a0;
  s.a = b.a;
  s.alpha0 = b.alpha0;
  s.rot = bi != B_PUCK;
  return s;
}
HK_HD void bodyAdvance(const Scene& S, Body& b, int bi, float alpha) {
  Sweep s = bodySweep(S, b, bi);
  sweepAdvance(s, alpha);
  b.c0 = s.c0;
  b.a0 = s.a0;
  b.alpha0 = s.alpha0;
  b.c = b.c0;
  b.a = b.a0;
  b.q = rotForBody(bi, b.a);
  b.p = b.c - mul(b.q, s.lc);
}

HK_HD float slantedFaceGap(const Scene& S, int f, const AABB& b) {
  const int k = (f & 1) ? 1 : 3;
  const Poly& P = S.poly[f];
  const float nx = P.nx[k], ny = P.ny[k];
  const float px = P.vx[k] + S.spx[f], py = P.vy[k] + S.spy[f];
  const float cx = nx > 0.0f ? b.lx : b.hx, cy = ny > 0.0f ? b.ly : b.hy;
  return nx * (cx - px) + ny * (cy - py);
}

HK_HD bool toiProvablySeparated(const Scene& S, const Env& e, int pid, int fA, int bi, float radiusB) {
  const Body& B = e.b[bi];
  V2 dc = B.c - B.c0;
  const bool known = sepKnown(e, pid);
  const float sepB = known ? e.sepBound[pid] : -HK_MAXFLOAT;
  const V2 sn = known ? e.sepNormal[pid] : mk(0.0f, 0.0f);
  float toward = (sn.x == 0.0f && sn.y == 0.0f) ? length(dc) : -dot(sn, dc);
  float disp = fmax2(toward, 0.0f) + (bi == B_PUCK ? 0.0f : 0.5f * fabs2(B.a - B.a0));
  float totalRadius = HK_POLYGON_RADIUS + radiusB;
  float target = fmax2(HK_LINEAR_SLOP, totalRadius - 3.0f * HK_LINEAR_SLOP);
  if (sepB - disp > target + 0.25f * HK_LINEAR_SLOP + 0.002f) return true;
  float da = fabs2(B.a - B.a0);
  if (bi != B_PUCK && da > 0.2f) return false;
  float sag = bi == B_PUCK ? 0.0f : 0.0625f * da * da;
  if (bi != B_PUCK && !(sn.x == 0.0f && sn.y == 0.0f) && sepB > 0.0f) {
    const Poly& PA = S.poly[fA];
    int k = -1;
    for (int i = 0; i < PA.count; ++i)
      if (PA.nx[i] == sn.x && PA.ny[i] == sn.y) k = i;
    if (k >= 0) {
      const Poly& PB = S.poly[F_R1 + bi];
      const Xf xfB = bodyXf(B);
      const float px = PA.vx[k] + S.spx[fA], py = PA.vy[k] + S.spy[fA];
      float sEnd = HK_MAXFLOAT;
      for (int i = 0; i < PB.count; ++i) {
        V2 v = mul(xfB, polyV(PB, i));
        sEnd = fmin2(sEnd, sn.x * (v.x - px) + sn.y * (v.y - py));
      }
      if (fmin2(sepB, sEnd) - sag - 0.001f > target + 0.25f * HK_LINEAR_SLOP + 0.002f) return true;
    }
  }
  AABB st = S.sfat[fA];
  const float d = HK_AABB_EXTENSION + HK_POLYGON_RADIUS;
  st.lx += d; st.ly += d; st.hx -= d; st.hy -= d;
  AABB mv = e.swept[bi];
  mv.lx += radiusB; mv.ly += radiusB; mv.hx -= radiusB; mv.hy -= radiusB;
  float gx = fmax2(st.lx - mv.hx, mv.lx - st.hx), gy = fmax2(st.ly - mv.hy, mv.ly - st.hy);
  float gap = fmax2(gx, gy);
  if (fA >= 2 && fA < 6) gap = fmax2(gap, slantedFaceGap(S, fA, mv));
  return gap > target + 0.25f * HK_LINEAR_SLOP + sag + 0.005f;
}

HK_HD bool toiSeparatedAfterEvent(const Scene& S, const Env& e, int pid, int bi, float radiusB, V2 atC, float atA) {
  const Body& B = e.b[bi];
  const bool puck = bi == B_PUCK;
  const V2 dc = B.c - B.c0;
  const V2 sn = e.sepNormal[pid];
  const float toward = (sn.x == 0.0f && sn.y == 0.0f) ? length(dc) : -dot(sn, dc);
  const float disp = fmax2(toward, 0.0f) + (puck ? 0.0f : 0.5f * fabs2(B.a - B.a0));
  const float corr = length(B.c0 - atC) + (puck ? 0.0f : 0.5f * fabs2(B.a0 - atA));
  const float totalRadius = HK_POLYGON_RADIUS + radiusB;
  const float target = fmax2(HK_LINEAR_SLOP, totalRadius - 3.0f * HK_LINEAR_SLOP);
  return sepBoundOf(e, pid) - corr - disp > target + 0.25f * HK_LINEAR_SLOP + 0.004f;
}

struct ToiTask {
  V2 c0, c;
  float a0, a;
  int pid;
};
HK_HD float toiTaskRun(const Scene& S, const ToiTask& t) {
  const int fA = S.pairFA[t.pid], fB = S.pairFB[t.pid];
  const int bi = fB - F_R1;
  Proxy pA, pB;
  pA.poly = &S.poly[fA];
  pA.radius = HK_POLYGON_RADIUS;
  if (fB == F_PUCK) {
    pB.poly = nullptr;
    pB.radius = S.puckRadius;
  } else {
    pB.poly = &S.poly[fB];
    pB.radius = HK_POLYGON_RADIUS;
  }
  Sweep sA;
  sA.lc = mk(0.0f, 0.0f);
  sA.c0 = sA.c = mk(S.spx[fA], S.spy[fA]);
  sA.a0 = sA.a = 0.0f;
  sA.alpha0 = 0.0f;
  sA.rot = false;
  Sweep sB;
  sB.lc = mk(S.lcx[bi], S.lcy[bi]);
  sB.c0 = t.c0;
  sB.c = t.c;
  sB.a0 = t.a0;
  sB.a = t.a;
  sB.alpha0 = 0.0f;
  sB.rot = bi != B_PUCK;
  int state;
  float tt;
  timeOfImpact(&state, &tt, pA, sA, pB, sB, 1.0f);
  const float alpha0 = 0.0f;
  return state == TOI_TOUCHING ? fmin2(alpha0 + (1.0f - alpha0) * tt, 1.0f) : 1.0f;
}
HK_HD int toiCollect(const Scene& S, Env& e, ToiTask* tasks, int maxTasks) {
  e.toiPreFlag = 0;
  int nt = 0;
  const uint32_t solvedMask = (e.b[0].island ? 1u : 0u) | (e.b[1].island ? 2u : 0u) | (e.b[2].island ? 4u : 0u);
  for (int i = 0; i < e.ncontacts; ++i) {
    int pid = clistGet(e.clist, i);
    uint32_t bit = 1u << pid;
    if (!(e.enabled & bit) || !(HK_PAIRS_TOI & bit)) continue;
    int fA = S.pairFA[pid], fB = S.pairFB[pid];
    int bi = fB - F_R1;
    const Body& B = e.b[bi];
    if (!B.awake) continue;
    float rB = fB == F_PUCK ? S.puckRadius : HK_POLYGON_RADIUS;
    if (((solvedMask >> bi) & 1u) && toiProvablySeparated(S, e, pid, fA, bi, rB)) {
      e.toiPre[pid] = 1.0f;
      e.toiPreFlag |= bit;
    } else if (nt < maxTasks) {
      ToiTask& t = tasks[nt++];
      t.c0 = B.c0;
      t.c = B.c;
      t.a0 = B.a0;
      t.a = B.a;
      t.pid = pid;
    }
  }
  return nt;
}

HK_HD_NOINLINE void solveTOI(const Scene& S, const Config& cfg, const Cache& cache, Env& e, float dt, int velIters) {
  HK_TOI_DBG(10);
  float salpha[8];
  for (int i = 0; i < 8; ++i) salpha[i] = 0.0f;
  const uint32_t solvedMask = (e.b[0].island ? 1u : 0u) | (e.b[1].island ? 2u : 0u) | (e.b[2].island ? 4u : 0u);
  e.b[0].island = e.b[1].island = e.b[2].island = false;
  e.b[0].alpha0 = e.b[1].alpha0 = e.b[2].alpha0 = 0.0f;
  uint32_t toiFlag = e.toiPreFlag;
  float* toi = e.toiPre;
  uint64_t toiCountLo = 0, toiCountHi = 0;
  e.toiPreFlag = 0;
  uint32_t freshMask = 0;
  int freshBody = -1;
  V2 freshC = mk(0.0f, 0.0f);
  float freshA = 0.0f;
  for (;;) {
    int minPid = -1;
    float minAlpha = 1.0f;
    for (int i = 0; i < e.ncontacts; ++i) {
      int pid = clistGet(e.clist, i);
      uint32_t bit = 1u << pid;
      if (!(e.enabled & bit)) continue;
      if ((int)(((pid < 16 ? toiCountLo : toiCountHi) >> (4 * (pid & 15))) & 15u) > HK_MAX_SUBSTEPS) continue;
      float alpha = 1.0f;
      if (toiFlag & bit) {
        alpha = toi[pid];
      } else {
        if (!(HK_PAIRS_TOI & bit)) continue;
        int fA = S.pairFA[pid], fB = S.pairFB[pid];
        int bi = fB - F_R1;
        Body& B = e.b[bi];
        if (!B.awake) continue;
        int sb = staticBodyOf(fA);
        float alpha0 = salpha[sb];
        if (salpha[sb] < B.alpha0) {
          alpha0 = B.alpha0;
          salpha[sb] = alpha0;
        } else if (B.alpha0 < salpha[sb]) {
          alpha0 = salpha[sb];
          Sweep s = bodySweep(S, B, bi);
          sweepAdvance(s, alpha0);
          B.c0 = s.c0;
          B.a0 = s.a0;
          B.alpha0 = s.alpha0;
        }
        Proxy pA, pB;
        pA.poly = &S.poly[fA];
        pA.radius = HK_POLYGON_RADIUS;
        if (fB == F_PUCK) {
          pB.poly = nullptr;
          pB.radius = S.puckRadius;
        } else {
          pB.poly = &S.poly[fB];
          pB.radius = HK_POLYGON_RADIUS;
        }
        Sweep sA;
        sA.lc = mk(0.0f, 0.0f);
        sA.c0 = sA.c = mk(S.spx[fA], S.spy[fA]);
        sA.a0 = sA.a = 0.0f;
        sA.alpha0 = salpha[sb];
        sA.rot = false;
        Sweep sB = bodySweep(S, B, bi);
        int state;
        float t;
        bool skip = !e.toiEventSeen && alpha0 == 0.0f && ((solvedMask >> bi) & 1u) &&
                    toiProvablySeparated(S, e, pid, fA, bi, pB.radius);
        if (!skip && bi == freshBody && (freshMask & bit) && sepKnown(e, pid))
          skip = toiSeparatedAfterEvent(S, e, pid, bi, pB.radius, freshC, freshA);
        HK_TOI_DBG(bi == B_PUCK ? 0 : 1);
        if (skip) {
          state = TOI_SEPARATED;
          t = 1.0f;
          HK_TOI_DBG(bi == B_PUCK ? 2 : 3);
        } else {
#if defined(__CUDA_ARCH__)
          long long c0_ = clock64();
#endif
          timeOfImpact(&state, &t, pA, sA, pB, sB, 1.0f);
#if defined(__CUDA_ARCH__)
          e.dbgEvalClk += clock64() - c0_;
#endif
          HK_TOI_DBG(bi == B_PUCK ? 4 : 5);
          if (e.toiEventSeen) HK_TOI_DBG(6);
          else if (!(alpha0 == 0.0f && ((solvedMask >> bi) & 1u))) HK_TOI_DBG(7);
          else if (!sepKnown(e, pid)) HK_TOI_DBG(8);
          if (state == TOI_TOUCHING) HK_TOI_DBG(9);
        }
        float beta = t;
        if (state == TOI_TOUCHING) alpha = fmin2(alpha0 + (1.0f - alpha0) * beta, 1.0f);
        else alpha = 1.0f;
        toi[pid] = alpha;
        toiFlag |= bit;
      }
      if (alpha < minAlpha) {
        minPid = pid;
        minAlpha = alpha;
      }
    }
    if (minPid < 0 || 1.0f - 10.0f * HK_EPS < minAlpha) break;
    if (!e.allowToiEvents) {
      e.aborted = true;
      return;
    }
    e.nToiEvents++;
    e.toiEventSeen = true;
#if defined(__CUDA_ARCH__)
    long long ev0_ = clock64();
#endif

    const int fA = S.pairFA[minPid], fB = S.pairFB[minPid];
    const int bi = fB - F_R1;
    const int sbA = staticBodyOf(fA);
    Body& B = e.b[bi];
    const Body backupB = B;
    const float backupSA = salpha[sbA];
    salpha[sbA] = minAlpha;
    bodyAdvance(S, B, bi, minAlpha);
    freshBody = bi;
    freshC = B.c;
    freshA = B.a;
    freshMask = 1u << minPid;
    updateContact(S, cfg, cache, e, minPid);
    toiFlag &= ~(1u << minPid);
    if (minPid < 16) toiCountLo += 1ull << (4 * minPid); else toiCountHi += 1ull << (4 * (minPid - 16));
    if (!(e.enabled & (1u << minPid)) || !(e.touch & (1u << minPid))) {
      e.enabled &= ~(1u << minPid);
      salpha[sbA] = backupSA;
      B.c0 = backupB.c0;
      B.c = backupB.c;
      B.a0 = backupB.a0;
      B.a = backupB.a;
      B.alpha0 = backupB.alpha0;
      syncTransform(S, B, bi);
      freshBody = -1;
      continue;
    }
    setAwake(B, true);
    int ic[MAX_MANIFOLDS];
    int nic = 0;
    ic[nic++] = minPid;
    uint32_t inIsland = 1u << minPid;
    uint32_t staticIsland = 1u << sbA;
    const uint32_t mine = bi == 0 ? HK_PAIRS_R1 : (bi == 1 ? HK_PAIRS_R2 : HK_PAIRS_PUCK);
    for (int i = 0; i < e.ncontacts; ++i) {
      int pid = clistGet(e.clist, i);
      uint32_t bit = 1u << pid;
      if (!(mine & bit)) continue;
      if (nic == MAX_MANIFOLDS) break;
      if (inIsland & bit) continue;
      if (!(HK_PAIRS_TOI & bit)) continue;
      int so = staticBodyOf(S.pairFA[pid]);
      float backup = salpha[so];
      if (!((staticIsland >> so) & 1u)) salpha[so] = minAlpha;
      updateContact(S, cfg, cache, e, pid);
      freshMask |= bit;
      if (!(e.enabled & bit) || !(e.touch & bit)) {
        salpha[so] = backup;
        continue;
      }
      inIsland |= bit;
      ic[nic++] = pid;
      staticIsland |= 1u << so;
    }
    const float subDt = (1.0f - minAlpha) * dt;
    for (int it = 0; it < 20; ++it) {
      float minSeparation = 0.0f;
      for (int k = 0; k < nic; ++k) {
        int slot = findSlot(e, ic[k]);
        if (slot < 0) continue;
        const Manifold& m = e.mf[slot];
        minSeparation = fmin2(minSeparation, solvePositionConstraint(S, e, ic[k], m, m.count, true));
      }
      if (minSeparation >= -1.5f * HK_LINEAR_SLOP) break;
    }
    B.c0 = B.c;
    B.a0 = B.a;
    VC vcs[MAX_MANIFOLDS];
    int nvc = 0;
    for (int k = 0; k < nic; ++k) {
      int slot = findSlot(e, ic[k]);
      if (slot < 0 || e.mf[slot].count == 0) continue;
      initConstraint(S, e, ic[k], slot, false, &vcs[nvc]);
      ++nvc;
    }
    int itc = runVelocityIterations(e, vcs, nvc, velIters);
    if (itc < 0) {
      e.aborted = true;
      return;
    }
    HK_ITER_HIST(1, itc);
    integratePosition(B, subDt);
    syncTransform(S, B, bi);
    B.island = false;
    synchronizeFixtures(S, e, bi);
    toiFlag &= ~mine;
    findNewContacts(S, e);
#if defined(__CUDA_ARCH__)
    e.dbgEventClk += clock64() - ev0_;
#endif
  }
}

HK_HD_NOINLINE void worldStepCollide(const Scene& S, const Config& cfg, const Cache& cache, Env& e) {
  e.enabled = 0xFFFFFFFFu;
  e.nmf = 0;
  e.toiEventSeen = false;
  e.toiPreFlag = 0;
  e.sepValid = 0;
  if (e.moved & 8u) {
    e.moved &= ~8u;
    findNewContacts(S, e);
  }
  collide(S, cfg, cache, e);
}
HK_HD void worldStepFinish(const Cache& cache, Env& e) {
  commitCache(cache, e);
  for (int bi = 0; bi < 3; ++bi) {
    e.b[bi].f = mk(0.0f, 0.0f);
    e.b[bi].tq = 0.0f;
  }
}
HK_HD_NOINLINE void worldStep(const Scene& S, const Config& cfg, const Cache& cache, Env& e, float dt, int velIters, int posIters) {
  worldStepCollide(S, cfg, cache, e);
  solveIslands(S, cfg, cache, e, dt, velIters, posIters);
  if (e.aborted) return;
  if (e.exist & HK_PAIRS_TOI) solveTOI(S, cfg, cache, e, dt, velIters);
  if (e.aborted) return;
  worldStepFinish(cache, e);
}

}
```

Baseline: 131.7 million.

## Pool TOI sweeps and TOI velocity solves across the block in lockstep rounds

Result: slower. 129.3 million, median of 6 (-1.8%).

```diff
diff --git a/hockey_env_b200/csrc/hk_lib.cu b/hockey_env_b200/csrc/hk_lib.cu
--- a/hockey_env_b200/csrc/hk_lib.cu
+++ b/hockey_env_b200/csrc/hk_lib.cu
@@ -356,6 +356,7 @@
 }
 struct GenStamps {
   long long tc0, tc1, tc2, tc3, stampB, stampV, stampT, tf0, tfCommit, tfFinish, tfStore, tfFlush;
+  unsigned toiRounds[4];
 };
 __device__ __forceinline__ long long clockAfterBarrier(const Scene& S) {
   const unsigned v = *reinterpret_cast<const volatile unsigned*>(&S.puckRadius);
@@ -368,51 +369,21 @@
   if (TEAM) asm volatile("bar.sync 2, %0;" ::"r"(nthr) : "memory");
   else __syncthreads();
 }
+template <bool TEAM>
+__device__ __forceinline__ bool teamAny(bool p, int nthr) {
+  if (!TEAM) return __syncthreads_or(p) != 0;
+  unsigned r;
+  asm volatile("{\n\t.reg .pred q, o;\n\tsetp.ne.u32 q, %1, 0;\n\tbar.red.or.pred o, 2, %2, q;\n\tselp.u32 %0, 1, 0, o;\n\t}"
+               : "=r"(r) : "r"((unsigned)p), "r"(nthr) : "memory");
+  return r != 0;
+}
 template <int TIER, bool TEAM>
-__device__ __forceinline__ void generalTick(const KParams& P, const StepIO& io, const Scene& S, unsigned char* sRaw, const bool valid,
-                                            const int64_t i, const int cls, const bool envWarp, const int64_t gw, const int unlimited,
-                                            const int phaseSync, const int envWarps, const int nthr, const bool laneWrite,
-                                            TickStats& st, bool& need, GenStamps& gs, unsigned long long* sSlowUnitP, unsigned* sFin) {
-  const int envLanes = envWarps << 5;
-  tickStatsZero(st);
-  need = false;
+__device__ __forceinline__ int pooledVelocitySolve(const KParams& P, const Scene& S, unsigned char* sRaw, Env& e, VC* vcs, const int nvc,
+                                                   const bool has, const int unlimited, const int phaseSync, const int envLanes, const int nthr,
+                                                   unsigned long long* sSlowUnitP, long long* stampB) {
   const int lane = threadIdx.x & 31;
   const int wib = threadIdx.x >> 5;
-  Env e;
-  Cache cache;
-  cache.base = P.cache + i;
-  cache.stride = (size_t)P.n;
-  int had1 = 0, had2 = 0;
-  const uint64_t env_id = (uint64_t)(P.env_id_offset + i);
-  const float dt = (float)(1.0 / HK_FPS);
-  long long& tc0 = gs.tc0; tc0 = clock64();
-  if (valid) {
-    loadEnv(P.core, P.n, i, e);
-    float a[8];
-    if (io.actBuf) {
-      const float4* ab = reinterpret_cast<const float4*>(io.actBuf + 8 * i);
-      float4 lo = ab[0], hi = ab[1];
-      a[0] = lo.x; a[1] = lo.y; a[2] = lo.z; a[3] = lo.w; a[4] = hi.x; a[5] = hi.y; a[6] = hi.z; a[7] = hi.w;
-      policyAdvancePhases(P.cfg, e, env_id, io.pol1, pol2Of(io, (size_t)i));
-    } else {
-      policyActions(P.cfg, e, env_id, io.action ? io.action + (size_t)io.stride * i : nullptr, io.pol1, pol2Of(io, (size_t)i), a);
-    }
-    had1 = e.has1;
-    had2 = e.has2;
-    e.sweepBudget = (TIER == 1 && !unlimited) ? kMidSweeps : (1 << 20);
-    e.allowToiEvents = TIER != 1 || unlimited;
-    e.aborted = false;
-    envStepActions(S, P.cfg, e, a);
-    worldStepCollide(S, P.cfg, cache, e);
-  }
-  const long long tw1 = clock64();
-  if (phaseSync & 1) teamSync<TEAM>(nthr);
-  long long& tc1 = gs.tc1; tc1 = clockAfterBarrier(S);
-  IslandCtx ctx;
-  ctx.nvc = 0;
-  long long &stampB = gs.stampB, &stampV = gs.stampV, &stampT = gs.stampT;
-  stampB = stampV = stampT = 0;
-  if (valid) solveIslandsBegin(S, cache, e, dt, ctx);
+  const bool trace = P.trace && sSlowUnitP;
   {
     SolveTask* mtasks = reinterpret_cast<SolveTask*>(sRaw);
     Solve2Task* s2tasks = reinterpret_cast<Solve2Task*>(sRaw + kRawMulti);
@@ -423,39 +394,39 @@
     __shared__ int sRound[5];
     if (threadIdx.x < HK_MULTI_KINDS + 3) sKindCount[threadIdx.x] = 0;
     if (threadIdx.x < 5) sRound[threadIdx.x] = 0;
-    if (threadIdx.x == 0) *sSlowUnitP = 0;
+    if (threadIdx.x == 0 && sSlowUnitP) *sSlowUnitP = 0;
     teamSync<TEAM>(nthr);
-    stampB = clockAfterBarrier(S);
+    if (stampB) *stampB = clockAfterBarrier(S);
     const int nwarps = nthr >> 5;
     const int budget = (TIER == 1 && !unlimited) ? kMidSweeps : (1 << 20);
     const bool pool1 = (phaseSync & 8) != 0;
     int kind = 0, slot = 0;
-    if (valid && ctx.nvc >= 2) {
-      kind = solveKind(ctx.vcs, ctx.nvc);
+    if (has && nvc >= 2) {
+      kind = solveKind(vcs, nvc);
       if (kind) {
         slot = atomicAdd(&sKindCount[HK_MULTI_KINDS + 2], 1);
         if (slot >= kMultiSlots) kind = 0;
         else atomicAdd(&sKindCount[kind - 1], 1);
       }
-    } else if (valid && ctx.nvc == 1 && pool1) {
-      kind = HK_MULTI_KINDS + ctx.vcs[0].count;
+    } else if (has && nvc == 1 && pool1) {
+      kind = HK_MULTI_KINDS + vcs[0].count;
       slot = atomicAdd(&sKindCount[kind - 1], 1);
       if (kind == HK_MULTI_KINDS + 2 && slot >= cap2) kind = 0;
     }
     if (kind == HK_MULTI_KINDS + 1) {
       Solve1Task& t = s1tasks[slot];
-      t.vc = vc1Of(ctx.vcs[0]);
-      t.A = loadVel(e, ctx.vcs[0].bA);
-      t.B = loadVel(e, ctx.vcs[0].bB);
+      t.vc = vc1Of(vcs[0]);
+      t.A = loadVel(e, vcs[0].bA);
+      t.B = loadVel(e, vcs[0].bB);
     } else if (kind == HK_MULTI_KINDS + 2) {
       Solve2Task& t = s2tasks[slot];
-      t.vc = ctx.vcs[0];
-      t.A = loadVel(e, ctx.vcs[0].bA);
-      t.B = loadVel(e, ctx.vcs[0].bB);
+      t.vc = vcs[0];
+      t.A = loadVel(e, vcs[0].bA);
+      t.B = loadVel(e, vcs[0].bB);
     } else if (kind) {
       SolveTask& t = mtasks[slot];
       t.kind = kind;
-      for (int k = 0; k < ctx.nvc; ++k) t.vcs[k] = ctx.vcs[k];
+      for (int k = 0; k < nvc; ++k) t.vcs[k] = vcs[k];
       t.v.b0 = loadVel(e, 0);
       t.v.b1 = loadVel(e, 1);
       t.v.b2 = loadVel(e, 2);
@@ -479,7 +450,7 @@
       const int uStride = (phaseSync & 16) ? max(wHeavy, 1) : nwarps;
       const bool heavyWarp = !(phaseSync & 16) || wib < wHeavy || nwarps == 1;
       for (int r = 0, u = wib; heavyWarp && u < units; ++r, u = r * uStride + ((r & 1) ? uStride - 1 - wib : wib)) {
-        const long long tu0 = P.trace ? clock64() : 0;
+        const long long tu0 = trace ? clock64() : 0;
         int utype = 10;
         if (u < nm) {
           utype = mk_[u];
@@ -519,10 +490,10 @@
           }
         }
         if (u >= nm && u < nm + c2) utype = 9;
-        if (P.trace && lane == 0) atomicMax(sSlowUnitP, ((unsigned long long)(clock64() - tu0) << 8) | (unsigned)utype);
+        if (trace && lane == 0) atomicMax(sSlowUnitP, ((unsigned long long)(clock64() - tu0) << 8) | (unsigned)utype);
       }
       if ((phaseSync & 16) && wib >= wHeavy) {
-        const long long tu0 = P.trace ? clock64() : 0;
+        const long long tu0 = trace ? clock64() : 0;
         const int w1 = nwarps - wHeavy, myw = wib - wHeavy;
         int nA = n1, it0 = 0;
         for (int r = 0; r < 4 && nA > 0; ++r) {
@@ -550,44 +521,43 @@
           nA = sRound[r + 1];
           it0 = stop;
         }
-        if (P.trace && lane == 0) atomicMax(sSlowUnitP, ((unsigned long long)(clock64() - tu0) << 8) | 10u);
+        if (trace && lane == 0) atomicMax(sSlowUnitP, ((unsigned long long)(clock64() - tu0) << 8) | 10u);
       }
     }
     int itc = 0;
     {
-      const long long tu0 = P.trace ? clock64() : 0;
-      const bool inPlace = valid && ctx.nvc > 0 && !kind;
-      if (inPlace) itc = runVelocityIterations(e, ctx.vcs, ctx.nvc, 6 * 30);
-      if (P.trace && __any_sync(0xffffffffu, inPlace) && lane == 0) atomicMax(sSlowUnitP, ((unsigned long long)(clock64() - tu0) << 8) | 11u);
+      const long long tu0 = trace ? clock64() : 0;
+      const bool inPlace = has && nvc > 0 && !kind;
+      if (inPlace) itc = runVelocityIterations(e, vcs, nvc, 6 * 30);
+      if (trace && __any_sync(0xffffffffu, inPlace) && lane == 0) atomicMax(sSlowUnitP, ((unsigned long long)(clock64() - tu0) << 8) | 11u);
     }
     teamSync<TEAM>(nthr);
-    stampV = clockAfterBarrier(S);
     if (kind == HK_MULTI_KINDS + 1) {
       const Solve1Task& t = s1tasks[slot];
-      ctx.vcs[0].pt[0].ni = t.vc.ni;
-      ctx.vcs[0].pt[0].ti = t.vc.ti;
-      storeVel(e, ctx.vcs[0].bA, t.A);
-      storeVel(e, ctx.vcs[0].bB, t.B);
+      vcs[0].pt[0].ni = t.vc.ni;
+      vcs[0].pt[0].ti = t.vc.ti;
+      storeVel(e, vcs[0].bA, t.A);
+      storeVel(e, vcs[0].bB, t.B);
       e.nVelIters += (uint32_t)t.sweeps;
       itc = t.result;
     } else if (kind == HK_MULTI_KINDS + 2) {
       const Solve2Task& t = s2tasks[slot];
-      ctx.vcs[0].pt[0].ni = t.vc.pt[0].ni;
-      ctx.vcs[0].pt[0].ti = t.vc.pt[0].ti;
-      ctx.vcs[0].pt[1].ni = t.vc.pt[1].ni;
-      ctx.vcs[0].pt[1].ti = t.vc.pt[1].ti;
-      storeVel(e, ctx.vcs[0].bA, t.A);
-      storeVel(e, ctx.vcs[0].bB, t.B);
+      vcs[0].pt[0].ni = t.vc.pt[0].ni;
+      vcs[0].pt[0].ti = t.vc.pt[0].ti;
+      vcs[0].pt[1].ni = t.vc.pt[1].ni;
+      vcs[0].pt[1].ti = t.vc.pt[1].ti;
+      storeVel(e, vcs[0].bA, t.A);
+      storeVel(e, vcs[0].bB, t.B);
       e.nVelIters += (uint32_t)t.sweeps;
       itc = t.result;
     } else if (kind) {
       const SolveTask& t = mtasks[slot];
-      for (int k = 0; k < ctx.nvc; ++k) {
-        ctx.vcs[k].pt[0].ni = t.vcs[k].pt[0].ni;
-        ctx.vcs[k].pt[0].ti = t.vcs[k].pt[0].ti;
-        if (ctx.vcs[k].count == 2) {
-          ctx.vcs[k].pt[1].ni = t.vcs[k].pt[1].ni;
-          ctx.vcs[k].pt[1].ti = t.vcs[k].pt[1].ti;
+      for (int k = 0; k < nvc; ++k) {
+        vcs[k].pt[0].ni = t.vcs[k].pt[0].ni;
+        vcs[k].pt[0].ti = t.vcs[k].pt[0].ti;
+        if (vcs[k].count == 2) {
+          vcs[k].pt[1].ni = t.vcs[k].pt[1].ni;
+          vcs[k].pt[1].ti = t.vcs[k].pt[1].ti;
         }
       }
       storeVel(e, 0, t.v.b0);
@@ -596,6 +566,57 @@
       e.nVelIters += (uint32_t)t.sweeps;
       itc = t.result;
     }
+    return itc;
+  }
+}
+template <int TIER, bool TEAM>
+__device__ __forceinline__ void generalTick(const KParams& P, const StepIO& io, const Scene& S, unsigned char* sRaw, const bool valid,
+                                            const int64_t i, const int cls, const bool envWarp, const int64_t gw, const int unlimited,
+                                            const int phaseSync, const int envWarps, const int nthr, const bool laneWrite,
+                                            TickStats& st, bool& need, GenStamps& gs, unsigned long long* sSlowUnitP, unsigned* sFin) {
+  const int envLanes = envWarps << 5;
+  tickStatsZero(st);
+  need = false;
+  const int lane = threadIdx.x & 31;
+  const int wib = threadIdx.x >> 5;
+  Env e;
+  Cache cache;
+  cache.base = P.cache + i;
+  cache.stride = (size_t)P.n;
+  int had1 = 0, had2 = 0;
+  const uint64_t env_id = (uint64_t)(P.env_id_offset + i);
+  const float dt = (float)(1.0 / HK_FPS);
+  long long& tc0 = gs.tc0; tc0 = clock64();
+  if (valid) {
+    loadEnv(P.core, P.n, i, e);
+    float a[8];
+    if (io.actBuf) {
+      const float4* ab = reinterpret_cast<const float4*>(io.actBuf + 8 * i);
+      float4 lo = ab[0], hi = ab[1];
+      a[0] = lo.x; a[1] = lo.y; a[2] = lo.z; a[3] = lo.w; a[4] = hi.x; a[5] = hi.y; a[6] = hi.z; a[7] = hi.w;
+      policyAdvancePhases(P.cfg, e, env_id, io.pol1, pol2Of(io, (size_t)i));
+    } else {
+      policyActions(P.cfg, e, env_id, io.action ? io.action + (size_t)io.stride * i : nullptr, io.pol1, pol2Of(io, (size_t)i), a);
+    }
+    had1 = e.has1;
+    had2 = e.has2;
+    e.sweepBudget = (TIER == 1 && !unlimited) ? kMidSweeps : (1 << 20);
+    e.allowToiEvents = TIER != 1 || unlimited;
+    e.aborted = false;
+    envStepActions(S, P.cfg, e, a);
+    worldStepCollide(S, P.cfg, cache, e);
+  }
+  const long long tw1 = clock64();
+  if (phaseSync & 1) teamSync<TEAM>(nthr);
+  long long& tc1 = gs.tc1; tc1 = clockAfterBarrier(S);
+  IslandCtx ctx;
+  ctx.nvc = 0;
+  long long &stampB = gs.stampB, &stampV = gs.stampV, &stampT = gs.stampT;
+  stampB = stampV = stampT = 0;
+  if (valid) solveIslandsBegin(S, cache, e, dt, ctx);
+  {
+    const int itc = pooledVelocitySolve<TIER, TEAM>(P, S, sRaw, e, ctx.vcs, ctx.nvc, valid, unlimited, phaseSync, envLanes, nthr, sSlowUnitP, &stampB);
+    stampV = clockAfterBarrier(S);
     if (valid) solveIslandsEnd(S, e, dt, 2 * 30, ctx, itc);
   }
   const long long tw2 = clock64();
@@ -629,7 +650,56 @@
     }
   }
   const long long tw3a = clock64();
-  if (wantToi) solveTOI(S, P.cfg, cache, e, dt, 6 * 30);
+  ToiLoop L;
+  for (int k = 0; k < 4; ++k) gs.toiRounds[k] = 0;
+  if (phaseSync & 32) {
+    ToiTask* sTasks = reinterpret_cast<ToiTask*>(sRaw);
+    float* sBeta = reinterpret_cast<float*>(sRaw + sizeof(ToiTask) * (size_t)envLanes * kTasksPerLane);
+    __shared__ int sCount3;
+    __shared__ unsigned sRoundStat[4];
+    if (threadIdx.x == 0) sCount3 = 0;
+    if (P.trace && threadIdx.x < 4) sRoundStat[threadIdx.x] = 0;
+    bool active = wantToi;
+    if (active) toiBegin(e, L);
+    const int nwarps = nthr >> 5;
+    while (teamAny<TEAM>(active, nthr)) {
+      const long long tr0 = P.trace ? clock64() : 0;
+      ToiTask mine[kTasksPerLane];
+      const int nMine = active ? toiScan(S, e, L, mine, kTasksPerLane) : 0;
+      int base = 0;
+      if (nMine > 0) {
+        base = atomicAdd(&sCount3, nMine);
+        for (int k = 0; k < nMine; ++k) sTasks[base + k] = mine[k];
+      }
+      teamSync<TEAM>(nthr);
+      const int total = sCount3;
+      for (int t = lane * nwarps + wib; t < total; t += nthr) sBeta[t] = toiTaskBeta(S, sTasks[t]);
+      teamSync<TEAM>(nthr);
+      if (threadIdx.x == 0) sCount3 = 0;
+      toiResolve(e, mine, sBeta + base, nMine);
+      const int r = active ? toiEventBegin(S, P.cfg, cache, e, L, dt, ctx.vcs, &ctx.nvc) : TOI_DONE;
+      if (r == TOI_DONE) active = false;
+      const bool pooled = r == TOI_SOLVE && ctx.nvc > 0;
+      if (teamAny<TEAM>(pooled, nthr)) {
+        const int itc = pooledVelocitySolve<TIER, TEAM>(P, S, sRaw, e, ctx.vcs, ctx.nvc, pooled, unlimited, phaseSync, envLanes, nthr, nullptr, nullptr);
+        if (pooled) toiEventEnd(S, e, L, itc);
+      }
+      if (r == TOI_SOLVE && !pooled) toiEventEnd(S, e, L, runVelocityIterations(e, ctx.vcs, 0, 6 * 30));
+      if (e.aborted) active = false;
+      if (P.trace) {
+        if (r != TOI_DONE) atomicAdd(&sRoundStat[1], 1u);
+        if (threadIdx.x == 0) {
+          sRoundStat[0] += 1;
+          sRoundStat[2] += (unsigned)total;
+          sRoundStat[3] = max(sRoundStat[3], (unsigned)(clock64() - tr0));
+        }
+      }
+    }
+    if (P.trace && threadIdx.x == 0)
+      for (int k = 0; k < 4; ++k) gs.toiRounds[k] = sRoundStat[k];
+  } else if (wantToi) {
+    solveTOILane(S, P.cfg, cache, e, dt, 6 * 30, L, ctx.vcs);
+  }
   const long long tw3 = clock64();
   if (P.trace && TIER == 1 && envWarp && lane == 0 && gw < P.n / 32 + 8) {
     uint32_t* w = P.trace + 4 * (size_t)gw;
@@ -811,7 +881,7 @@
     if (__any_sync(1u, valid) || true) {
       long long tc4 = clockAfterBarrier(S);
       if (P.trace && TIER == 1 && blockIdx.x < P.n / 32 + 8) {
-        uint32_t* w = P.trace + 4 * ((size_t)P.n / 32 + 8) + 2 * (size_t)P.n + 16 * (size_t)blockIdx.x;
+        uint32_t* w = P.trace + 4 * ((size_t)P.n / 32 + 8) + 2 * (size_t)P.n + 20 * (size_t)blockIdx.x;
         w[0] = (uint32_t)(tc1 - tc0);
         w[1] = (uint32_t)(stampB - tc1);
         w[2] = (uint32_t)(stampV - stampB);
@@ -832,6 +902,7 @@
         w[13] = sFin[1];
         w[14] = sFin[2];
         w[15] = sFin[3];
+        for (int k = 0; k < 4; ++k) w[16 + k] = gs.toiRounds[k];
       }
       if (!P.trace && TIER == 1) {
         atomicAdd(&P.phaseClk[8], (unsigned long long)(gs.tf0 - tc3));
@@ -1285,7 +1356,7 @@
       shapeSharedMemory();
       g_shapedFor = shapeKey();
     }
-    if (trace) cudaMemsetAsync(trace, 0, sizeof(uint32_t) * (20 * ((size_t)n / 32 + 8) + 2 * (size_t)n), stream);
+    if (trace) cudaMemsetAsync(trace, 0, sizeof(uint32_t) * (24 * ((size_t)n / 32 + 8) + 2 * (size_t)n), stream);
     stamp(0, stream);
     if (fastWide) k_fast<1, kFastWide><<<(unsigned)((n + fastWideBlock - 1) / fastWideBlock), fastWideBlock, 0, stream>>>(params(), io);
     else if (n < 100000) k_fast<4, kBlock><<<(unsigned)((n + fastBlock - 1) / fastBlock), fastBlock, 0, stream>>>(params(), io);
@@ -1391,8 +1462,8 @@
     if (const char* fb = getenv("HK_FAST_BLOCK")) h->fastBlock = std::min(kBlock, std::max(32, atoi(fb) / 32 * 32));
     h->fastWide = n_envs >= 16000;
     if (const char* fw = getenv("HK_FAST_WIDE")) h->fastWide = fw[0] == '1';
-    h->phaseSync = 31;
-    if (const char* ps = getenv("HK_PHASE_SYNC")) h->phaseSync = atoi(ps) & 31;
+    h->phaseSync = n_envs >= 100000 ? 63 : 31;
+    if (const char* ps = getenv("HK_PHASE_SYNC")) h->phaseSync = atoi(ps) & 63;
     int sms = 148;
     if (cudaDeviceGetAttribute(&sms, cudaDevAttrMultiProcessorCount, device) != cudaSuccess || sms < 16) sms = 148;
     {
@@ -1430,7 +1501,7 @@
   if (err == cudaSuccess) err = cudaMalloc(&h->actBuf, sizeof(float) * 8 * (size_t)n_envs);
   if (err == cudaSuccess) err = cudaMalloc(&h->phaseClk, sizeof(unsigned long long) * 16);
   if (err == cudaSuccess) err = cudaMemset(h->phaseClk, 0, sizeof(unsigned long long) * 16);
-  if (err == cudaSuccess && getenv("HK_LANE_TRACE")) err = cudaMalloc(&h->trace, sizeof(uint32_t) * (20 * ((size_t)n_envs / 32 + 8) + 2 * (size_t)n_envs));
+  if (err == cudaSuccess && getenv("HK_LANE_TRACE")) err = cudaMalloc(&h->trace, sizeof(uint32_t) * (24 * ((size_t)n_envs / 32 + 8) + 2 * (size_t)n_envs));
   if (err == cudaSuccess) err = cudaMemset(h->cache, 0, sizeof(uint32_t) * 6 * N_PAIRS * (size_t)n_envs);
   if (err == cudaSuccess) err = cudaMemset(h->stats, 0, sizeof(double) * HK_STATS_DIM * (kStatsRows + 1));
   if (err == cudaSuccess) {
@@ -1793,7 +1864,7 @@
 int hk_debug_lane_trace(hk_env* h, uint32_t* out_host, int64_t n_words) {
   if (!h || !out_host) return fail(HK_E_INVALID, "hk_debug_lane_trace: NULL argument");
   if (!h->trace) return fail(HK_E_INVALID, "hk_debug_lane_trace: create the env with HK_LANE_TRACE=1");
-  const int64_t have = 20 * (h->n / 32 + 8) + 2 * h->n;
+  const int64_t have = 24 * (h->n / 32 + 8) + 2 * h->n;
   DeviceGuard guard(h->device);
   HK_CUDA(cudaMemcpy(out_host, h->trace, sizeof(uint32_t) * (size_t)(n_words < have ? n_words : have), cudaMemcpyDeviceToHost));
   return HK_OK;
diff --git a/hockey_env_b200/csrc/hk_world.cuh b/hockey_env_b200/csrc/hk_world.cuh
--- a/hockey_env_b200/csrc/hk_world.cuh
+++ b/hockey_env_b200/csrc/hk_world.cuh
@@ -1879,206 +1879,275 @@
   return nt;
 }
 
-HK_HD_NOINLINE void solveTOI(const Scene& S, const Config& cfg, const Cache& cache, Env& e, float dt, int velIters) {
+struct ToiLoop {
+  float salpha[8];
+  uint32_t solvedMask;
+  uint32_t toiFlag;
+  uint64_t toiCountLo, toiCountHi;
+  uint32_t freshMask;
+  int freshBody;
+  V2 freshC;
+  float freshA;
+  int bi;
+  float subDt;
+};
+HK_HD float toiTaskBeta(const Scene& S, const ToiTask& t) {
+  const int fA = S.pairFA[t.pid], fB = S.pairFB[t.pid];
+  const int bi = fB - F_R1;
+  Proxy pA, pB;
+  pA.poly = &S.poly[fA];
+  pA.radius = HK_POLYGON_RADIUS;
+  if (fB == F_PUCK) {
+    pB.poly = nullptr;
+    pB.radius = S.puckRadius;
+  } else {
+    pB.poly = &S.poly[fB];
+    pB.radius = HK_POLYGON_RADIUS;
+  }
+  Sweep sA;
+  sA.lc = mk(0.0f, 0.0f);
+  sA.c0 = sA.c = mk(S.spx[fA], S.spy[fA]);
+  sA.a0 = sA.a = 0.0f;
+  sA.alpha0 = 0.0f;
+  sA.rot = false;
+  Sweep sB;
+  sB.lc = mk(S.lcx[bi], S.lcy[bi]);
+  sB.c0 = t.c0;
+  sB.c = t.c;
+  sB.a0 = t.a0;
+  sB.a = t.a;
+  sB.alpha0 = 0.0f;
+  sB.rot = bi != B_PUCK;
+  int state;
+  float tt;
+  timeOfImpact(&state, &tt, pA, sA, pB, sB, 1.0f);
+  return state == TOI_TOUCHING ? tt : -1.0f;
+}
+HK_HD float toiAlpha(float alpha0, float beta) { return beta != -1.0f ? fmin2(alpha0 + (1.0f - alpha0) * beta, 1.0f) : 1.0f; }
+
+HK_HD void toiBegin(Env& e, ToiLoop& L) {
   HK_TOI_DBG(10);
-  float salpha[8];
-  for (int i = 0; i < 8; ++i) salpha[i] = 0.0f;
-  const uint32_t solvedMask = (e.b[0].island ? 1u : 0u) | (e.b[1].island ? 2u : 0u) | (e.b[2].island ? 4u : 0u);
+  for (int i = 0; i < 8; ++i) L.salpha[i] = 0.0f;
+  L.solvedMask = (e.b[0].island ? 1u : 0u) | (e.b[1].island ? 2u : 0u) | (e.b[2].island ? 4u : 0u);
   e.b[0].island = e.b[1].island = e.b[2].island = false;
   e.b[0].alpha0 = e.b[1].alpha0 = e.b[2].alpha0 = 0.0f;
-  uint32_t toiFlag = e.toiPreFlag;
+  L.toiFlag = e.toiPreFlag;
+  L.toiCountLo = L.toiCountHi = 0;
+  e.toiPreFlag = 0;
+  L.freshMask = 0;
+  L.freshBody = -1;
+  L.freshC = mk(0.0f, 0.0f);
+  L.freshA = 0.0f;
+}
+
+HK_HD_NOINLINE int toiScan(const Scene& S, Env& e, ToiLoop& L, ToiTask* tasks, int maxTasks) {
   float* toi = e.toiPre;
-  uint64_t toiCountLo = 0, toiCountHi = 0;
-  e.toiPreFlag = 0;
-  uint32_t freshMask = 0;
-  int freshBody = -1;
-  V2 freshC = mk(0.0f, 0.0f);
-  float freshA = 0.0f;
+  int nt = 0;
+  for (int i = 0; i < e.ncontacts; ++i) {
+    int pid = clistGet(e.clist, i);
+    uint32_t bit = 1u << pid;
+    if (!(e.enabled & bit)) continue;
+    if ((int)(((pid < 16 ? L.toiCountLo : L.toiCountHi) >> (4 * (pid & 15))) & 15u) > HK_MAX_SUBSTEPS) continue;
+    if (L.toiFlag & bit) continue;
+    if (!(HK_PAIRS_TOI & bit)) continue;
+    int fA = S.pairFA[pid], fB = S.pairFB[pid];
+    int bi = fB - F_R1;
+    Body& B = e.b[bi];
+    if (!B.awake) continue;
+    int sb = staticBodyOf(fA);
+    float alpha0 = L.salpha[sb];
+    if (L.salpha[sb] < B.alpha0) {
+      alpha0 = B.alpha0;
+      L.salpha[sb] = alpha0;
+    } else if (B.alpha0 < L.salpha[sb]) {
+      alpha0 = L.salpha[sb];
+      Sweep s = bodySweep(S, B, bi);
+      sweepAdvance(s, alpha0);
+      B.c0 = s.c0;
+      B.a0 = s.a0;
+      B.alpha0 = s.alpha0;
+    }
+    const float radiusB = fB == F_PUCK ? S.puckRadius : HK_POLYGON_RADIUS;
+    bool skip = !e.toiEventSeen && alpha0 == 0.0f && ((L.solvedMask >> bi) & 1u) && toiProvablySeparated(S, e, pid, fA, bi, radiusB);
+    if (!skip && bi == L.freshBody && (L.freshMask & bit) && sepKnown(e, pid))
+      skip = toiSeparatedAfterEvent(S, e, pid, bi, radiusB, L.freshC, L.freshA);
+    HK_TOI_DBG(bi == B_PUCK ? 0 : 1);
+    ToiTask t;
+    t.c0 = B.c0;
+    t.c = B.c;
+    t.a0 = B.a0;
+    t.a = B.a;
+    t.pid = pid;
+    if (skip) {
+      toi[pid] = 1.0f;
+      HK_TOI_DBG(bi == B_PUCK ? 2 : 3);
+    } else if (nt < maxTasks) {
+      tasks[nt++] = t;
+      toi[pid] = alpha0;
+    } else {
+#if defined(__CUDA_ARCH__)
+      long long c0_ = clock64();
+#endif
+      const float beta = toiTaskBeta(S, t);
+      toi[pid] = toiAlpha(alpha0, beta);
+#if defined(__CUDA_ARCH__)
+      e.dbgEvalClk += clock64() - c0_;
+#endif
+      HK_TOI_DBG(bi == B_PUCK ? 4 : 5);
+      if (e.toiEventSeen) HK_TOI_DBG(6);
+      else if (!(alpha0 == 0.0f && ((L.solvedMask >> bi) & 1u))) HK_TOI_DBG(7);
+      else if (!sepKnown(e, pid)) HK_TOI_DBG(8);
+      if (beta != -1.0f) HK_TOI_DBG(9);
+    }
+    L.toiFlag |= bit;
+  }
+  return nt;
+}
+HK_HD void toiResolve(Env& e, const ToiTask* tasks, const float* beta, int nt) {
+  for (int k = 0; k < nt; ++k) e.toiPre[tasks[k].pid] = toiAlpha(e.toiPre[tasks[k].pid], beta[k]);
+}
+
+enum { TOI_DONE = 0, TOI_SOLVE = 1, TOI_DROPPED = 2 };
+HK_HD_NOINLINE int toiEventBegin(const Scene& S, const Config& cfg, const Cache& cache, Env& e, ToiLoop& L, float dt, VC* vcs, int* nvc) {
+  int minPid = -1;
+  float minAlpha = 1.0f;
+  for (int i = 0; i < e.ncontacts; ++i) {
+    int pid = clistGet(e.clist, i);
+    uint32_t bit = 1u << pid;
+    if (!(e.enabled & bit) || !(L.toiFlag & bit)) continue;
+    if ((int)(((pid < 16 ? L.toiCountLo : L.toiCountHi) >> (4 * (pid & 15))) & 15u) > HK_MAX_SUBSTEPS) continue;
+    const float alpha = e.toiPre[pid];
+    if (alpha < minAlpha) {
+      minPid = pid;
+      minAlpha = alpha;
+    }
+  }
+  if (minPid < 0 || 1.0f - 10.0f * HK_EPS < minAlpha) return TOI_DONE;
+  if (!e.allowToiEvents) {
+    e.aborted = true;
+    return TOI_DONE;
+  }
+  e.nToiEvents++;
+  e.toiEventSeen = true;
+
+  const int fA = S.pairFA[minPid], fB = S.pairFB[minPid];
+  const int bi = fB - F_R1;
+  const int sbA = staticBodyOf(fA);
+  float* salpha = L.salpha;
+  Body& B = e.b[bi];
+  const Body backupB = B;
+  const float backupSA = salpha[sbA];
+  salpha[sbA] = minAlpha;
+  bodyAdvance(S, B, bi, minAlpha);
+  L.freshBody = bi;
+  L.freshC = B.c;
+  L.freshA = B.a;
+  L.freshMask = 1u << minPid;
+  updateContact(S, cfg, cache, e, minPid);
+  L.toiFlag &= ~(1u << minPid);
+  if (minPid < 16) L.toiCountLo += 1ull << (4 * minPid); else L.toiCountHi += 1ull << (4 * (minPid - 16));
+  if (!(e.enabled & (1u << minPid)) || !(e.touch & (1u << minPid))) {
+    e.enabled &= ~(1u << minPid);
+    salpha[sbA] = backupSA;
+    B.c0 = backupB.c0;
+    B.c = backupB.c;
+    B.a0 = backupB.a0;
+    B.a = backupB.a;
+    B.alpha0 = backupB.alpha0;
+    syncTransform(S, B, bi);
+    L.freshBody = -1;
+    return TOI_DROPPED;
+  }
+  setAwake(B, true);
+  int ic[MAX_MANIFOLDS];
+  int nic = 0;
+  ic[nic++] = minPid;
+  uint32_t inIsland = 1u << minPid;
+  uint32_t staticIsland = 1u << sbA;
+  const uint32_t mine = bi == 0 ? HK_PAIRS_R1 : (bi == 1 ? HK_PAIRS_R2 : HK_PAIRS_PUCK);
+  for (int i = 0; i < e.ncontacts; ++i) {
+    int pid = clistGet(e.clist, i);
+    uint32_t bit = 1u << pid;
+    if (!(mine & bit)) continue;
+    if (nic == MAX_MANIFOLDS) break;
+    if (inIsland & bit) continue;
+    if (!(HK_PAIRS_TOI & bit)) continue;
+    int so = staticBodyOf(S.pairFA[pid]);
+    float backup = salpha[so];
+    if (!((staticIsland >> so) & 1u)) salpha[so] = minAlpha;
+    updateContact(S, cfg, cache, e, pid);
+    L.freshMask |= bit;
+    if (!(e.enabled & bit) || !(e.touch & bit)) {
+      salpha[so] = backup;
+      continue;
+    }
+    inIsland |= bit;
+    ic[nic++] = pid;
+    staticIsland |= 1u << so;
+  }
+  L.bi = bi;
+  L.subDt = (1.0f - minAlpha) * dt;
+  for (int it = 0; it < 20; ++it) {
+    float minSeparation = 0.0f;
+    for (int k = 0; k < nic; ++k) {
+      int slot = findSlot(e, ic[k]);
+      if (slot < 0) continue;
+      const Manifold& m = e.mf[slot];
+      minSeparation = fmin2(minSeparation, solvePositionConstraint(S, e, ic[k], m, m.count, true));
+    }
+    if (minSeparation >= -1.5f * HK_LINEAR_SLOP) break;
+  }
+  B.c0 = B.c;
+  B.a0 = B.a;
+  int n = 0;
+  for (int k = 0; k < nic; ++k) {
+    int slot = findSlot(e, ic[k]);
+    if (slot < 0 || e.mf[slot].count == 0) continue;
+    initConstraint(S, e, ic[k], slot, false, &vcs[n]);
+    ++n;
+  }
+  *nvc = n;
+  return TOI_SOLVE;
+}
+HK_HD_NOINLINE void toiEventEnd(const Scene& S, Env& e, ToiLoop& L, int itc) {
+  if (itc < 0) {
+    e.aborted = true;
+    return;
+  }
+  HK_ITER_HIST(1, itc);
+  const int bi = L.bi;
+  Body& B = e.b[bi];
+  integratePosition(B, L.subDt);
+  syncTransform(S, B, bi);
+  B.island = false;
+  synchronizeFixtures(S, e, bi);
+  L.toiFlag &= ~(bi == 0 ? HK_PAIRS_R1 : (bi == 1 ? HK_PAIRS_R2 : HK_PAIRS_PUCK));
+  findNewContacts(S, e);
+}
+
+HK_HD_NOINLINE void solveTOILane(const Scene& S, const Config& cfg, const Cache& cache, Env& e, float dt, int velIters, ToiLoop& L, VC* vcs) {
+  toiBegin(e, L);
   for (;;) {
-    int minPid = -1;
-    float minAlpha = 1.0f;
-    for (int i = 0; i < e.ncontacts; ++i) {
-      int pid = clistGet(e.clist, i);
-      uint32_t bit = 1u << pid;
-      if (!(e.enabled & bit)) continue;
-      if ((int)(((pid < 16 ? toiCountLo : toiCountHi) >> (4 * (pid & 15))) & 15u) > HK_MAX_SUBSTEPS) continue;
-      float alpha = 1.0f;
-      if (toiFlag & bit) {
-        alpha = toi[pid];
-      } else {
-        if (!(HK_PAIRS_TOI & bit)) continue;
-        int fA = S.pairFA[pid], fB = S.pairFB[pid];
-        int bi = fB - F_R1;
-        Body& B = e.b[bi];
-        if (!B.awake) continue;
-        int sb = staticBodyOf(fA);
-        float alpha0 = salpha[sb];
-        if (salpha[sb] < B.alpha0) {
-          alpha0 = B.alpha0;
-          salpha[sb] = alpha0;
-        } else if (B.alpha0 < salpha[sb]) {
-          alpha0 = salpha[sb];
-          Sweep s = bodySweep(S, B, bi);
-          sweepAdvance(s, alpha0);
-          B.c0 = s.c0;
-          B.a0 = s.a0;
-          B.alpha0 = s.alpha0;
-        }
-        Proxy pA, pB;
-        pA.poly = &S.poly[fA];
-        pA.radius = HK_POLYGON_RADIUS;
-        if (fB == F_PUCK) {
-          pB.poly = nullptr;
-          pB.radius = S.puckRadius;
-        } else {
-          pB.poly = &S.poly[fB];
-          pB.radius = HK_POLYGON_RADIUS;
-        }
-        Sweep sA;
-        sA.lc = mk(0.0f, 0.0f);
-        sA.c0 = sA.c = mk(S.spx[fA], S.spy[fA]);
-        sA.a0 = sA.a = 0.0f;
-        sA.alpha0 = salpha[sb];
-        sA.rot = false;
-        Sweep sB = bodySweep(S, B, bi);
-        int state;
-        float t;
-        bool skip = !e.toiEventSeen && alpha0 == 0.0f && ((solvedMask >> bi) & 1u) &&
-                    toiProvablySeparated(S, e, pid, fA, bi, pB.radius);
-        if (!skip && bi == freshBody && (freshMask & bit) && sepKnown(e, pid))
-          skip = toiSeparatedAfterEvent(S, e, pid, bi, pB.radius, freshC, freshA);
-        HK_TOI_DBG(bi == B_PUCK ? 0 : 1);
-        if (skip) {
-          state = TOI_SEPARATED;
-          t = 1.0f;
-          HK_TOI_DBG(bi == B_PUCK ? 2 : 3);
-        } else {
-#if defined(__CUDA_ARCH__)
-          long long c0_ = clock64();
-#endif
-          timeOfImpact(&state, &t, pA, sA, pB, sB, 1.0f);
-#if defined(__CUDA_ARCH__)
-          e.dbgEvalClk += clock64() - c0_;
-#endif
-          HK_TOI_DBG(bi == B_PUCK ? 4 : 5);
-          if (e.toiEventSeen) HK_TOI_DBG(6);
-          else if (!(alpha0 == 0.0f && ((solvedMask >> bi) & 1u))) HK_TOI_DBG(7);
-          else if (!sepKnown(e, pid)) HK_TOI_DBG(8);
-          if (state == TOI_TOUCHING) HK_TOI_DBG(9);
-        }
-        float beta = t;
-        if (state == TOI_TOUCHING) alpha = fmin2(alpha0 + (1.0f - alpha0) * beta, 1.0f);
-        else alpha = 1.0f;
-        toi[pid] = alpha;
-        toiFlag |= bit;
-      }
-      if (alpha < minAlpha) {
-        minPid = pid;
-        minAlpha = alpha;
-      }
-    }
-    if (minPid < 0 || 1.0f - 10.0f * HK_EPS < minAlpha) break;
-    if (!e.allowToiEvents) {
-      e.aborted = true;
-      return;
-    }
-    e.nToiEvents++;
-    e.toiEventSeen = true;
+    toiScan(S, e, L, nullptr, 0);
 #if defined(__CUDA_ARCH__)
     long long ev0_ = clock64();
 #endif
-
-    const int fA = S.pairFA[minPid], fB = S.pairFB[minPid];
-    const int bi = fB - F_R1;
-    const int sbA = staticBodyOf(fA);
-    Body& B = e.b[bi];
-    const Body backupB = B;
-    const float backupSA = salpha[sbA];
-    salpha[sbA] = minAlpha;
-    bodyAdvance(S, B, bi, minAlpha);
-    freshBody = bi;
-    freshC = B.c;
-    freshA = B.a;
-    freshMask = 1u << minPid;
-    updateContact(S, cfg, cache, e, minPid);
-    toiFlag &= ~(1u << minPid);
-    if (minPid < 16) toiCountLo += 1ull << (4 * minPid); else toiCountHi += 1ull << (4 * (minPid - 16));
-    if (!(e.enabled & (1u << minPid)) || !(e.touch & (1u << minPid))) {
-      e.enabled &= ~(1u << minPid);
-      salpha[sbA] = backupSA;
-      B.c0 = backupB.c0;
-      B.c = backupB.c;
-      B.a0 = backupB.a0;
-      B.a = backupB.a;
-      B.alpha0 = backupB.alpha0;
-      syncTransform(S, B, bi);
-      freshBody = -1;
-      continue;
-    }
-    setAwake(B, true);
-    int ic[MAX_MANIFOLDS];
-    int nic = 0;
-    ic[nic++] = minPid;
-    uint32_t inIsland = 1u << minPid;
-    uint32_t staticIsland = 1u << sbA;
-    const uint32_t mine = bi == 0 ? HK_PAIRS_R1 : (bi == 1 ? HK_PAIRS_R2 : HK_PAIRS_PUCK);
-    for (int i = 0; i < e.ncontacts; ++i) {
-      int pid = clistGet(e.clist, i);
-      uint32_t bit = 1u << pid;
-      if (!(mine & bit)) continue;
-      if (nic == MAX_MANIFOLDS) break;
-      if (inIsland & bit) continue;
-      if (!(HK_PAIRS_TOI & bit)) continue;
-      int so = staticBodyOf(S.pairFA[pid]);
-      float backup = salpha[so];
-      if (!((staticIsland >> so) & 1u)) salpha[so] = minAlpha;
-      updateContact(S, cfg, cache, e, pid);
-      freshMask |= bit;
-      if (!(e.enabled & bit) || !(e.touch & bit)) {
-        salpha[so] = backup;
-        continue;
-      }
-      inIsland |= bit;
-      ic[nic++] = pid;
-      staticIsland |= 1u << so;
-    }
-    const float subDt = (1.0f - minAlpha) * dt;
-    for (int it = 0; it < 20; ++it) {
-      float minSeparation = 0.0f;
-      for (int k = 0; k < nic; ++k) {
-        int slot = findSlot(e, ic[k]);
-        if (slot < 0) continue;
-        const Manifold& m = e.mf[slot];
-        minSeparation = fmin2(minSeparation, solvePositionConstraint(S, e, ic[k], m, m.count, true));
-      }
-      if (minSeparation >= -1.5f * HK_LINEAR_SLOP) break;
-    }
-    B.c0 = B.c;
-    B.a0 = B.a;
-    VC vcs[MAX_MANIFOLDS];
     int nvc = 0;
-    for (int k = 0; k < nic; ++k) {
-      int slot = findSlot(e, ic[k]);
-      if (slot < 0 || e.mf[slot].count == 0) continue;
-      initConstraint(S, e, ic[k], slot, false, &vcs[nvc]);
-      ++nvc;
-    }
-    int itc = runVelocityIterations(e, vcs, nvc, velIters);
-    if (itc < 0) {
-      e.aborted = true;
-      return;
-    }
-    HK_ITER_HIST(1, itc);
-    integratePosition(B, subDt);
-    syncTransform(S, B, bi);
-    B.island = false;
-    synchronizeFixtures(S, e, bi);
-    toiFlag &= ~mine;
-    findNewContacts(S, e);
+    const int r = toiEventBegin(S, cfg, cache, e, L, dt, vcs, &nvc);
+    if (r == TOI_DONE) return;
+    if (r == TOI_SOLVE) {
+      toiEventEnd(S, e, L, runVelocityIterations(e, vcs, nvc, velIters));
+      if (e.aborted) return;
+    }
 #if defined(__CUDA_ARCH__)
     e.dbgEventClk += clock64() - ev0_;
 #endif
   }
+}
+HK_HD void solveTOI(const Scene& S, const Config& cfg, const Cache& cache, Env& e, float dt, int velIters) {
+  ToiLoop L;
+  VC vcs[MAX_MANIFOLDS];
+  solveTOILane(S, cfg, cache, e, dt, velIters, L, vcs);
 }
 
 HK_HD_NOINLINE void worldStepCollide(const Scene& S, const Config& cfg, const Cache& cache, Env& e) {
```
